# yoraish/mmd

Hardware: AMD Instinct MI355X
Metric: guided trajectories/sec (H=64, 100 denoise steps), 32-robot Empty map (higher is better)
Workload: dtype f32 (f16x2 split on the fp16 MFMA pipe: every fp32 product as 3 fp16 MFMAs, fp32 accumulate)

## Files before the change

### include/mmd_amd.h

```cpp
#ifndef MMD_AMD_H
#define MMD_AMD_H

#include <stddef.h>
#include <stdint.h>

#ifdef __cplusplus
extern "C" {
#endif

#define MMD_AMD_ABI_VERSION 9
#define MMD_STATE_DIM 4
#define MMD_HORIZON 64

typedef struct mmd_unet_s* mmd_unet_t;

int mmd_abi_version(void);
const char* mmd_last_error(void);


int mmd_unet_num_tensors(int unet_input_dim, int n_levels);
int64_t mmd_unet_tensor_numel(int unet_input_dim, int n_levels, int index);

typedef struct mmd_unet_options {
  uint32_t flags;
// ... 17 lines not shown
int mmd_unet_forward(mmd_unet_t unet, const float* x_dev, int t, float* eps_dev, int n_traj, void* workspace_dev,
                     size_t workspace_bytes, void* stream);


typedef struct mmd_cons_bins {
  float lo[2], inv_cell[2];
  int32_t nx, ny, n_all, robot0;
  float radius, weight;
  const int32_t* cell_off_dev;
  const float* entries_dev;
} mmd_cons_bins;

typedef struct mmd_guide_desc {
  float norm_min[MMD_STATE_DIM];
  float norm_max[MMD_STATE_DIM];
  float limits_lo[2];
  float limits_hi[2];
  int32_t grid_nx, grid_ny, n_grids, n_maps;
  const float* sdf_grids_dev;
  const int32_t* robot_map_dev;
  float ws_min[2];
  float ws_max[2];
  float margin;
  float dt;
  float sigma_gp;
  float weight_collision;
  float weight_smoothness;
  float max_grad_norm;
  const float* cons_ell_dev;
  const int32_t* grp_slot_off_dev;
  const float* grp_weight_dev;
  const int32_t* robot_grp_off_dev;
  int32_t max_slots_per_robot;
  float cons_uniform_radius;
  const float* extra_spheres_dev;
  const float* extra_boxes_dev;
  int32_t n_extra_spheres, n_extra_boxes;
  int32_t clip_grad_rule;
  float max_grad_value;
  const mmd_cons_bins* cons_bins;
} mmd_guide_desc;

int mmd_pack_constraints(int n_groups, const int32_t* n_pts, const float* const* q, const float* const* t_range,
                         const float* const* radius, int horizon, float* ell_out, int max_slots,
                         int32_t* slots_out);

int mmd_soft_constraints_from_paths(const float* paths_dev, int n_all, int robot0, int n_local, int horizon,
                                    float radius, float weight, float* ell_out_dev, int32_t* grp_slot_off_dev,
                                    float* grp_weight_dev, int32_t* robot_grp_off_dev, void* stream);

size_t mmd_cons_bins_bytes(int n_all, int nx, int ny, size_t* off_bytes, size_t* entry_bytes);
int mmd_bin_constraints_from_paths(const float* paths_dev, int n_all, int horizon, float radius, const float lo[2], const float hi[2],
                                   int nx, int ny, int32_t* cell_off_dev, float* entries_dev, void* stream);

int mmd_bin_paths(const float* paths_dev, int n_all, int horizon, float reach, const float lo[2], const float hi[2], int nx, int ny,
                  int first_step, int32_t* cell_off_dev, float* entries_dev, void* stream);

int mmd_guide_steps(const mmd_guide_desc* g, float* x_dev, const float* hard_dev, uint64_t hard_rows, int n_robots,
                    int samples_per_robot, int n_steps, float* chain_dev, void* stream);


typedef struct mmd_sampler_desc {
  int32_t n_diffusion_steps;
  const float* sqrt_recip_alphas_cumprod;
  const float* sqrt_recipm1_alphas_cumprod;
  const float* posterior_mean_coef1;
  const float* posterior_mean_coef2;
  const float* posterior_log_variance_clipped;
  int32_t n_guide_steps;
  int32_t t_start_guide;
  float noise_std_extra;
  uint64_t hard_rows;
  int32_t n_streams;
  int64_t traj_index_base;
  const float* noise_std_extra_by_t;
  void* profiler;
  int32_t scale_grad_by_std;
  int32_t model_predicts_x0;
  uint32_t flags;
  int32_t guide_coop_max;
  const uint64_t* robot_seeds_dev;
} mmd_sampler_desc;
#define MMD_SAMPLER_NO_FUSED_STEP 1u
#define MMD_SAMPLER_PERSIST 2u

size_t mmd_sampler_workspace_bytes(mmd_unet_t unet, int n_traj);

int mmd_ddpm_step(mmd_unet_t unet, const mmd_sampler_desc* s, const mmd_guide_desc* guide, float* x_dev,
                  const float* hard_dev, int n_robots, int samples_per_robot, int i, const float* noise_dev,
                  uint64_t seed, uint32_t draw_index, void* workspace_dev, size_t workspace_bytes, void* stream);

int mmd_p_sample_loop(mmd_unet_t unet, const mmd_sampler_desc* s, const mmd_guide_desc* guide, float* x_dev,
                      const float* hard_dev, int n_robots, int samples_per_robot, int n_steps,
                      int n_steps_without_noise, int init_noise, const float* step_noise_dev, uint64_t seed,
                      float* chain_dev, void* workspace_dev, size_t workspace_bytes, void* stream);

int mmd_ddim_sample(mmd_unet_t unet, const mmd_sampler_desc* s, const float* alphas_cumprod, const int32_t* times,
                    int n_times, const mmd_guide_desc* guide, float* x_dev, const float* hard_dev, int n_robots,
                    int samples_per_robot, int init_noise, uint64_t seed, float* chain_dev, void* workspace_dev,
                    size_t workspace_bytes, void* stream);

int mmd_q_sample(float* x_dev, const float* x_start_dev, const float* noise_dev, float sqrt_alphas_cumprod_t,
                 float sqrt_one_minus_alphas_cumprod_t, uint64_t seed, uint32_t draw_index, int64_t traj_index_base,
                 int n_traj, void* stream);

int mmd_cross_condition(float* x1_dev, float* x2_dev, int ind1, int ind2, const float* rel, const float* boundary,
                        int n_traj, void* stream);

typedef struct mmd_ensemble_tile {
  mmd_unet_t unet;
  const mmd_sampler_desc* sampler;
  const mmd_guide_desc* guide;
  float* x_dev;
  const float* hard_dev;
  const float* step_noise_dev;
  float* chain_dev;
  uint64_t seed;
} mmd_ensemble_tile;

typedef struct mmd_cross_cond {
  int32_t m1, m2, ind1, ind2;
  float rel[4];
  float boundary[4];
  const float* by_robot_dev;
} mmd_cross_cond;

int mmd_p_sample_loop_ensemble(const mmd_ensemble_tile* tiles, int n_tiles, const mmd_cross_cond* cross, int n_cross,
                               int n_robots, int samples_per_robot, int n_steps, int n_steps_without_noise,
                               int init_noise, void* workspace_dev, size_t workspace_bytes, void* stream);


int mmd_rr_collisions(const float* paths_dev, int n_robots, int horizon, float margin, uint8_t* mask_dev,
                      float* midpoints_dev, void* stream);

int mmd_count_collisions(const float* trajs_dev, const float* paths_dev, int robot0, int n_local,
                         int samples_per_robot, int n_all, int horizon, float margin, int32_t* counts_dev, void* stream);

int mmd_count_collisions_binned(const float* trajs_dev, const mmd_cons_bins* bins, int n_local, int samples_per_robot, float margin,
                                int32_t* counts_dev, void* stream);

typedef struct mmd_agent_path {
  const float* batch_dev;
  int32_t index;
  int32_t length;
  int32_t start_time;
  int32_t reserved;
} mmd_agent_path;

typedef struct mmd_conflict {
  int32_t t, a, b, reserved;
  float pa[2], pb[2];
  float mid[2];
  float reserved2[2];
} mmd_conflict;

#define MMD_CONFLICTS_ORDERED 0
#define MMD_CONFLICTS_PAIRS 1
#define MMD_SELECT_CBS 0
#define MMD_SELECT_PP 1

int mmd_find_conflicts(const mmd_agent_path* agents_dev, int n_agents, int horizon_global, float margin, int mode,
                       int32_t* row_counts_dev, int32_t* count_dev, mmd_conflict* first_dev, mmd_conflict* list_dev, int list_cap,
                       void* stream);

int mmd_path_conflicts_binned(const float* paths_dev, const mmd_cons_bins* bins, int horizon, float margin, int32_t* row_counts_dev,
                              int32_t* robot_counts_dev, int32_t* count_dev, mmd_conflict* first_dev, mmd_conflict* list_dev, int list_cap,
// ... 62 lines not shown
```

### mmd_amd/_lib.py

```python
import ctypes as C
import os

_HERE = os.path.dirname(os.path.abspath(__file__))
LIB_PATH = os.path.join(_HERE, "lib", "libmmd_amd.so")
ABI_VERSION = 9
HARD_ROWS_START_GOAL = (1 << 63) | 1


def signed64(mask):
    mask = int(mask) & 0xFFFFFFFFFFFFFFFF
    return mask - (1 << 64) if mask >> 63 else mask



class ConsBins(C.Structure):
    _fields_ = [
        ("lo", C.c_float * 2), ("inv_cell", C.c_float * 2),
        ("nx", C.c_int32), ("ny", C.c_int32), ("n_all", C.c_int32), ("robot0", C.c_int32),
        ("radius", C.c_float), ("weight", C.c_float),
        ("cell_off_dev", C.c_void_p), ("entries_dev", C.c_void_p),
    ]


class GuideDesc(C.Structure):
    _fields_ = [
        ("norm_min", C.c_float * 4), ("norm_max", C.c_float * 4),
        ("limits_lo", C.c_float * 2), ("limits_hi", C.c_float * 2),
        ("grid_nx", C.c_int32), ("grid_ny", C.c_int32), ("n_grids", C.c_int32), ("n_maps", C.c_int32),
        ("sdf_grids_dev", C.c_void_p), ("robot_map_dev", C.c_void_p),
        ("ws_min", C.c_float * 2), ("ws_max", C.c_float * 2),
        ("margin", C.c_float), ("dt", C.c_float), ("sigma_gp", C.c_float),
        ("weight_collision", C.c_float), ("weight_smoothness", C.c_float), ("max_grad_norm", C.c_float),
        ("cons_ell_dev", C.c_void_p), ("grp_slot_off_dev", C.c_void_p), ("grp_weight_dev", C.c_void_p),
        ("robot_grp_off_dev", C.c_void_p), ("max_slots_per_robot", C.c_int32), ("cons_uniform_radius", C.c_float),
        ("extra_spheres_dev", C.c_void_p), ("extra_boxes_dev", C.c_void_p),
        ("n_extra_spheres", C.c_int32), ("n_extra_boxes", C.c_int32),
        ("clip_grad_rule", C.c_int32), ("max_grad_value", C.c_float),
        ("cons_bins", C.POINTER(ConsBins)),
    ]


class SamplerDesc(C.Structure):
    _fields_ = [
        ("n_diffusion_steps", C.c_int32),
        ("sqrt_recip_alphas_cumprod", C.POINTER(C.c_float)),
        ("sqrt_recipm1_alphas_cumprod", C.POINTER(C.c_float)),
        ("posterior_mean_coef1", C.POINTER(C.c_float)),
        ("posterior_mean_coef2", C.POINTER(C.c_float)),
        ("posterior_log_variance_clipped", C.POINTER(C.c_float)),
        ("n_guide_steps", C.c_int32), ("t_start_guide", C.c_int32),
        ("noise_std_extra", C.c_float), ("hard_rows", C.c_uint64), ("n_streams", C.c_int32),
        ("traj_index_base", C.c_int64), ("noise_std_extra_by_t", C.POINTER(C.c_float)), ("profiler", C.c_void_p),
        ("scale_grad_by_std", C.c_int32), ("model_predicts_x0", C.c_int32),
        ("flags", C.c_uint32), ("guide_coop_max", C.c_int32), ("robot_seeds_dev", C.c_void_p),
    ]


SAMPLER_NO_FUSED_STEP, SAMPLER_PERSIST = 1, 2
UNET_LAYERED, UNET_LAYERED_VALU = 1, 2
UNET_PRECISION_F32, UNET_PRECISION_F16 = 0, 1
UNET_PRECISIONS = {"f32": UNET_PRECISION_F32, "f16": UNET_PRECISION_F16}


class UnetOptions(C.Structure):
    _fields_ = [("flags", C.c_uint32), ("rtb_fused", C.c_int32), ("mconv_max_cs", C.c_int32), ("two_per_workgroup_max", C.c_int32),
                ("precision", C.c_int32)]


class EnsembleTile(C.Structure):
    _fields_ = [
        ("unet", C.c_void_p), ("sampler", C.POINTER(SamplerDesc)), ("guide", C.POINTER(GuideDesc)),
        ("x_dev", C.c_void_p), ("hard_dev", C.c_void_p), ("step_noise_dev", C.c_void_p), ("chain_dev", C.c_void_p),
        ("seed", C.c_uint64),
    ]


class CrossCond(C.Structure):
    _fields_ = [("m1", C.c_int32), ("m2", C.c_int32), ("ind1", C.c_int32), ("ind2", C.c_int32),
                ("rel", C.c_float * 4), ("boundary", C.c_float * 4), ("by_robot_dev", C.c_void_p)]


class AgentPath(C.Structure):
    _fields_ = [("batch_dev", C.c_void_p), ("index", C.c_int32), ("length", C.c_int32), ("start_time", C.c_int32),
                ("reserved", C.c_int32)]


class Conflict(C.Structure):
    _fields_ = [("t", C.c_int32), ("a", C.c_int32), ("b", C.c_int32), ("reserved", C.c_int32), ("pa", C.c_float * 2),
                ("pb", C.c_float * 2), ("mid", C.c_float * 2), ("reserved2", C.c_float * 2)]


class TileRef(C.Structure):
    _fields_ = [("agent", C.c_int32), ("t0", C.c_int32), ("offset", C.c_float * 2), ("rule", C.c_int32), ("reserved", C.c_int32)]


ADHERENCE_LINE, ADHERENCE_HIGHWAYS, ADHERENCE_CONVEYOR, ADHERENCE_DROP_REGION = 0, 1, 2, 3
CONFLICTS_ORDERED, CONFLICTS_PAIRS = 0, 1
SELECT_CBS, SELECT_PP = 0, 1


_SIGNATURES = {
    "mmd_abi_version": (C.c_int, []),
    "mmd_last_error": (C.c_char_p, []),
    "mmd_unet_num_tensors": (C.c_int, [C.c_int, C.c_int]),
    "mmd_unet_tensor_numel": (C.c_int64, [C.c_int, C.c_int, C.c_int]),
    "mmd_unet_create": (C.c_int, [C.POINTER(C.c_void_p), C.c_int, C.c_int, C.c_int, C.POINTER(C.c_void_p),
                                  C.POINTER(C.c_int64), C.c_int, C.POINTER(UnetOptions), C.c_void_p]),
    "mmd_unet_destroy": (C.c_int, [C.c_void_p]),
    "mmd_unet_workspace_bytes": (C.c_size_t, [C.c_void_p, C.c_int]),
    "mmd_unet_forward": (C.c_int, [C.c_void_p, C.c_void_p, C.c_int, C.c_void_p, C.c_int, C.c_void_p, C.c_size_t,
                                   C.c_void_p]),
    "mmd_pack_constraints": (C.c_int, [C.c_int, C.POINTER(C.c_int32), C.POINTER(C.c_void_p), C.POINTER(C.c_void_p),
                                       C.POINTER(C.c_void_p), C.c_int, C.c_void_p, C.c_int, C.POINTER(C.c_int32)]),
    "mmd_soft_constraints_from_paths": (C.c_int, [C.c_void_p, C.c_int, C.c_int, C.c_int, C.c_int, C.c_float, C.c_float,
                                                  C.c_void_p, C.c_void_p, C.c_void_p, C.c_void_p, C.c_void_p]),
    "mmd_cons_bins_bytes": (C.c_size_t, [C.c_int, C.c_int, C.c_int, C.POINTER(C.c_size_t), C.POINTER(C.c_size_t)]),
    "mmd_bin_constraints_from_paths": (C.c_int, [C.c_void_p, C.c_int, C.c_int, C.c_float, C.POINTER(C.c_float), C.POINTER(C.c_float),
                                                 C.c_int, C.c_int, C.c_void_p, C.c_void_p, C.c_void_p]),
    "mmd_bin_paths": (C.c_int, [C.c_void_p, C.c_int, C.c_int, C.c_float, C.POINTER(C.c_float), C.POINTER(C.c_float), C.c_int, C.c_int,
                                C.c_int, C.c_void_p, C.c_void_p, C.c_void_p]),
    "mmd_guide_steps": (C.c_int, [C.POINTER(GuideDesc), C.c_void_p, C.c_void_p, C.c_uint64, C.c_int, C.c_int, C.c_int,
                                  C.c_void_p, C.c_void_p]),
    "mmd_sampler_workspace_bytes": (C.c_size_t, [C.c_void_p, C.c_int]),
    "mmd_ddpm_step": (C.c_int, [C.c_void_p, C.POINTER(SamplerDesc), C.POINTER(GuideDesc), C.c_void_p, C.c_void_p,
                                C.c_int, C.c_int, C.c_int, C.c_void_p, C.c_uint64, C.c_uint32, C.c_void_p, C.c_size_t,
                                C.c_void_p]),
    "mmd_p_sample_loop": (C.c_int, [C.c_void_p, C.POINTER(SamplerDesc), C.POINTER(GuideDesc), C.c_void_p, C.c_void_p,
                                    C.c_int, C.c_int, C.c_int, C.c_int, C.c_int, C.c_void_p, C.c_uint64, C.c_void_p,
                                    C.c_void_p, C.c_size_t, C.c_void_p]),
    "mmd_ddim_sample": (C.c_int, [C.c_void_p, C.POINTER(SamplerDesc), C.c_void_p, C.c_void_p, C.c_int, C.POINTER(GuideDesc),
                                  C.c_void_p, C.c_void_p, C.c_int, C.c_int, C.c_int, C.c_uint64, C.c_void_p, C.c_void_p,
                                  C.c_size_t, C.c_void_p]),
    "mmd_p_sample_loop_ensemble": (C.c_int, [C.POINTER(EnsembleTile), C.c_int, C.POINTER(CrossCond), C.c_int, C.c_int,
                                             C.c_int, C.c_int, C.c_int, C.c_int, C.c_void_p, C.c_size_t, C.c_void_p]),
    "mmd_q_sample": (C.c_int, [C.c_void_p, C.c_void_p, C.c_void_p, C.c_float, C.c_float, C.c_uint64, C.c_uint32,
                               C.c_int64, C.c_int, C.c_void_p]),
    "mmd_rr_collisions": (C.c_int, [C.c_void_p, C.c_int, C.c_int, C.c_float, C.c_void_p, C.c_void_p, C.c_void_p]),
    "mmd_count_collisions": (C.c_int, [C.c_void_p, C.c_void_p, C.c_int, C.c_int, C.c_int, C.c_int, C.c_int, C.c_float,
                                       C.c_void_p, C.c_void_p]),
    "mmd_count_collisions_binned": (C.c_int, [C.c_void_p, C.POINTER(ConsBins), C.c_int, C.c_int, C.c_float, C.c_void_p, C.c_void_p]),
    "mmd_path_conflicts_binned": (C.c_int, [C.c_void_p, C.POINTER(ConsBins), C.c_int, C.c_float, C.c_void_p, C.c_void_p, C.c_void_p,
# ... 109 lines not shown
```

### mmd_amd/csrc/api.hip

```cpp
#include <hip/hip_runtime.h>

#include <cmath>
#include <cstdarg>
#include <cstdio>
#include <cstdlib>
#include <map>
#include <vector>

#include "../../include/mmd_amd.h"
#include "../../include/mmd_amd_debug.h"
#include "common.h"
#include "guide_dev.h"

struct mmd_profiler_s {
  int stride = 1, window = 1, period = 0;
  std::vector<hipEvent_t> ev;
  std::vector<int> kind;
  hipEvent_t base = nullptr;
  size_t used = 0;
  size_t seen[2] = {0, 0};
};

namespace mmd {

// ... 30 lines not shown
  int nch = n_streams;
  if (nch <= 0) nch = (long long)n_robots * samples_per_robot > 512 ? 2 : 1;
  if (nch > kMaxChunks) nch = kMaxChunks;
  if (nch > n_robots) nch = n_robots;
  return nch < 1 ? 1 : nch;
}


struct Streams {
  hipStream_t s[kMaxChunks] = {};
  hipEvent_t fork = nullptr, join[kMaxChunks] = {};
  bool tried = false, good = false;
  bool ok() {
    if (!tried) {
      tried = true;
      good = hipEventCreateWithFlags(&fork, hipEventDisableTiming) == hipSuccess;
      for (int c = 0; c < kMaxChunks && good; ++c)
        good = hipStreamCreateWithFlags(&s[c], hipStreamNonBlocking) == hipSuccess &&
               hipEventCreateWithFlags(&join[c], hipEventDisableTiming) == hipSuccess;
    }
    return good;
  }
};
static Streams& streams() {
  static thread_local std::map<int, Streams> S;
  int dev = 0;
  (void)hipGetDevice(&dev);
  return S[dev];
}

static StepDev step_base(const mmd_sampler_desc* s) {
  StepDev sd{};
  sd.do_model = 1;
  sd.n_guide_steps = s->n_guide_steps;
  sd.hard_rows = s->hard_rows; sd.n_hard = __builtin_popcountll(s->hard_rows);
  sd.traj_base = (long long)s->traj_index_base;
  return sd;
}

static int make_step(const mmd_sampler_desc* s, int i, bool guided, StepDev& sd) {
  const int t = i < 0 ? 0 : i;
  MMD_REQUIRE(t < s->n_diffusion_steps, "loop index %d outside the %d-step schedule", i, s->n_diffusion_steps);
  sd = step_base(s);
  sd.a_t = s->sqrt_recip_alphas_cumprod[t];
  sd.b_t = s->sqrt_recipm1_alphas_cumprod[t];
  if (s->model_predicts_x0) { sd.a_t = 0.f; sd.b_t = -1.f; }
  sd.grad_scale = s->scale_grad_by_std ? expf(s->posterior_log_variance_clipped[t]) : 1.f;
  sd.c1 = s->posterior_mean_coef1[t];
  sd.c2 = s->posterior_mean_coef2[t];
  sd.sigma = expf(0.5f * s->posterior_log_variance_clipped[t]);
  sd.noise_std_extra = s->noise_std_extra_by_t ? s->noise_std_extra_by_t[t] : s->noise_std_extra;
  sd.do_guide = guided && i < s->t_start_guide ? 1 : 0;
  sd.do_noise = t == 0 ? 0 : 1;
  sd.robot_seeds = reinterpret_cast<const unsigned long long*>(s->robot_seeds_dev);
  sd.coop_max = s->guide_coop_max;
  return 0;
}

static StepDev make_ddim_step(const mmd_sampler_desc* s, const float* alphas_cumprod, int t, int tn, bool guided) {
  StepDev sd = step_base(s);
  sd.ddim = s->model_predicts_x0 ? 2 : 1;
  sd.grad_scale = 1.f;
  sd.a_t = s->sqrt_recip_alphas_cumprod[t];
  sd.b_t = s->model_predicts_x0 ? (tn < 0 ? 0.f : 1.f / s->sqrt_recipm1_alphas_cumprod[t]) : s->sqrt_recipm1_alphas_cumprod[t];
  sd.c1 = tn < 0 ? 1.f : sqrtf(alphas_cumprod[tn]);
  sd.c2 = tn < 0 ? 0.f : sqrtf(1.f - alphas_cumprod[tn]);
  sd.do_guide = guided && tn >= 0 && tn < s->t_start_guide ? 1 : 0;
  sd.do_noise = 0;
  return sd;
}

static FusedStep fused_step(const StepDev& sd, float* x, const float* hard, const float* noise, float* chain, int traj0, int spr,
                            int t_row = 0) {
  FusedStep fs{};
  fs.enabled = 1;
  fs.a_t = sd.a_t; fs.b_t = sd.b_t; fs.c1 = sd.c1; fs.c2 = sd.c2; fs.sigma = sd.sigma; fs.noise_std_extra = sd.noise_std_extra;
  fs.do_noise = sd.do_noise; fs.hard_rows = sd.hard_rows; fs.n_hard = sd.n_hard; fs.seed = sd.seed; fs.draw = sd.draw;
  fs.robot_seeds = sd.robot_seeds;
  fs.traj_base = sd.traj_base; fs.traj0 = traj0; fs.spr = spr;
  fs.x = reinterpret_cast<float4*>(x); fs.noise = reinterpret_cast<const float4*>(noise);
  fs.chain = reinterpret_cast<float4*>(chain); fs.hard = reinterpret_cast<const float4*>(hard);
  fs.t_row = t_row;
  return fs;
}

static int bins_of(const mmd_guide_desc* guide, const mmd_sampler_desc* s, const mmd_cons_bins** out) {
  *out = guide ? guide->cons_bins : nullptr;
  MMD_REQUIRE(!(*out && s->robot_seeds_dev), "cons_bins with per-robot seeds (robot_seeds_dev: batched planner calls) is not supported");
  return 0;
}

template <class T>
static inline T* row_of(T* buf, size_t k, size_t traj_floats) { return buf ? buf + k * traj_floats : nullptr; }

static inline float* eps_of(void* workspace_dev, mmd_unet_t unet, int n) {
  return reinterpret_cast<float*>(reinterpret_cast<char*>(workspace_dev) + mmd_unet_workspace_bytes(unet, n));
}

static int ddpm_step(mmd_unet_t unet, const mmd_sampler_desc* s, const mmd_guide_desc* guide, float* x_dev, const float* hard_dev, int n,
                     int samples_per_robot, int i, const float* noise_dev, uint64_t seed, uint32_t draw_index, void* workspace_dev,
                     mmd_profiler_t prof, float* mu_dev, float* guide_chain_dev, uint32_t* trace_dev, void* stream) {
  StepDev sd{};
  if (int rc = make_step(s, i, guide != nullptr, sd)) return rc;
  sd.seed = seed; sd.draw = draw_index;
  const mmd_cons_bins* bins = nullptr;
  if (int rc = bins_of(guide, s, &bins)) return rc;
  if (trace_dev) {
    MMD_REQUIRE(!bins, "mmd_debug_ddpm_step_trace: the decision dump reads the ELL table, not a cell table (cons_bins)");
    MMD_REQUIRE(sd.do_guide, "mmd_debug_ddpm_step_trace: step %d is not a guided one (t_start_guide %d)", i, s->t_start_guide);
    sd.guide_chain = reinterpret_cast<float4*>(guide_chain_dev);
    sd.guide_chain_stride = (long long)n * H;
    sd.trace = trace_dev;
    sd.mu_out = reinterpret_cast<float4*>(mu_dev);
  }
  GuideDev g{};
  if (sd.do_guide)
    if (int rc = fill_guide(guide, g)) return rc;
  float* eps = eps_of(workspace_dev, unet, n);
  if (int rc = mmd_unet_forward_profiled(unet, x_dev, i < 0 ? 0 : i, eps, n, workspace_dev, mmd_unet_workspace_bytes(unet, n), prof, stream))
    return rc;
  launch_step(g, sd, x_dev, eps, noise_dev, nullptr, hard_dev, 0, n, samples_per_robot, (hipStream_t)stream, bins);
  MMD_HIP_CHECK(hipGetLastError());
  return 0;
}

}

using namespace mmd;

extern "C" {

int mmd_abi_version(void) { return MMD_AMD_ABI_VERSION; }
int mmd_sampler_stream_chunks(int n_streams, int n_robots, int samples_per_robot) {
  return stream_chunks(n_streams, n_robots, samples_per_robot);
}
const char* mmd_last_error(void) { return g_err; }

size_t mmd_sampler_workspace_bytes(mmd_unet_t unet, int n_traj) {
  return mmd_unet_workspace_bytes(unet, n_traj) + (size_t)(n_traj > 0 ? n_traj : 0) * H * D * sizeof(float);
}

int mmd_ddpm_step(mmd_unet_t unet, const mmd_sampler_desc* s, const mmd_guide_desc* guide, float* x_dev,
                  const float* hard_dev, int n_robots, int samples_per_robot, int i, const float* noise_dev,
                  uint64_t seed, uint32_t draw_index, void* workspace_dev, size_t workspace_bytes, void* stream) {
  MMD_REQUIRE(unet && s && x_dev && hard_dev && workspace_dev, "mmd_ddpm_step: NULL argument");
  const int n = n_robots * samples_per_robot;
  MMD_REQUIRE(n >= 1, "mmd_ddpm_step: empty batch");
  MMD_REQUIRE(workspace_bytes >= mmd_sampler_workspace_bytes(unet, n), "mmd_ddpm_step: workspace too small");
  return ddpm_step(unet, s, guide, x_dev, hard_dev, n, samples_per_robot, i, noise_dev, seed, draw_index, workspace_dev,
                   (mmd_profiler_t)s->profiler, nullptr, nullptr, nullptr, stream);
}

int mmd_debug_ddpm_step_trace(mmd_unet_t unet, const mmd_sampler_desc* s, const mmd_guide_desc* guide, float* x_dev,
                              const float* hard_dev, int n_robots, int samples_per_robot, int i, const float* noise_dev,
                              uint64_t seed, uint32_t draw_index, void* workspace_dev, size_t workspace_bytes,
                              float* mu_dev, float* guide_chain_dev, uint32_t* trace_dev, void* stream) {
  MMD_REQUIRE(unet && s && guide && x_dev && hard_dev && workspace_dev && guide_chain_dev && trace_dev,
              "mmd_debug_ddpm_step_trace: NULL argument");
  const int n = n_robots * samples_per_robot;
  MMD_REQUIRE(n >= 1, "mmd_debug_ddpm_step_trace: empty batch");
  MMD_REQUIRE(workspace_bytes >= mmd_sampler_workspace_bytes(unet, n), "mmd_debug_ddpm_step_trace: workspace too small");
  return ddpm_step(unet, s, guide, x_dev, hard_dev, n, samples_per_robot, i, noise_dev, seed, draw_index, workspace_dev, nullptr,
                   mu_dev, guide_chain_dev, trace_dev, stream);
}

int mmd_p_sample_loop(mmd_unet_t unet, const mmd_sampler_desc* s, const mmd_guide_desc* guide, float* x_dev,
                      const float* hard_dev, int n_robots, int samples_per_robot, int n_steps,
                      int n_steps_without_noise, int init_noise, const float* step_noise_dev, uint64_t seed,
                      float* chain_dev, void* workspace_dev, size_t workspace_bytes, void* stream) {
  MMD_REQUIRE(unet && s && x_dev && hard_dev && workspace_dev, "mmd_p_sample_loop: NULL argument");
  const int n = n_robots * samples_per_robot;
  MMD_REQUIRE(n >= 1, "mmd_p_sample_loop: empty batch");
  MMD_REQUIRE(n_steps >= 0 && n_steps <= s->n_diffusion_steps && n_steps_without_noise >= 0, "bad step counts");
  MMD_REQUIRE(workspace_bytes >= mmd_sampler_workspace_bytes(unet, n), "mmd_p_sample_loop: workspace too small");
  hipStream_t st = (hipStream_t)stream;
  const size_t traj_floats = (size_t)n * H * D;
  GuideDev g{};
  if (guide)
    if (int rc = fill_guide(guide, g)) return rc;
  const mmd_cons_bins* bins = nullptr;
  if (int rc = bins_of(guide, s, &bins)) return rc;
  launch_init(x_dev, chain_dev, hard_dev, s->hard_rows, init_noise, (unsigned long long)seed,
              reinterpret_cast<const unsigned long long*>(s->robot_seeds_dev), (long long)s->traj_index_base, n, samples_per_robot, st);
  const bool persist = (s->flags & MMD_SAMPLER_PERSIST) != 0, no_fused_step = (s->flags & MMD_SAMPLER_NO_FUSED_STEP) != 0;
  const mmd_profiler_t prof = (mmd_profiler_t)s->profiler;

  int k_start = 0;
  hipStreamCaptureStatus capturing = hipStreamCaptureStatusNone;
  if (persist) (void)hipStreamIsCapturing(st, &capturing);
  if (persist && capturing == hipStreamCaptureStatusNone && !no_fused_step && unet_fused_step_supported(unet) && !prof) {
    FusedStep run[PERSIST_MAX_STEPS];
    int i = n_steps - 1, k0 = 0;
    while (i >= -n_steps_without_noise) {
      int m = 0;
      for (; m < PERSIST_MAX_STEPS && i - m >= -n_steps_without_noise; ++m) {
        StepDev sd{};
        if (int rc = make_step(s, i - m, guide != nullptr, sd)) return rc;
        if (sd.do_guide) break;
        sd.seed = seed; sd.draw = (unsigned int)(k0 + m);
        run[m] = fused_step(sd, x_dev, hard_dev, row_of(step_noise_dev, k0 + m, traj_floats), row_of(chain_dev, k0 + m + 1, traj_floats), 0,
                            samples_per_robot, i - m < 0 ? 0 : i - m);
      }
      if (m == 0 || (m < 2 && k0 == 0)) break;
      if (int rc = unet_persist_steps(unet, n, workspace_dev, mmd_unet_workspace_bytes(unet, n), st, run, m)) return rc;
      k0 += m; i -= m;
    }
    k_start = k0;
  }
  int nch = stream_chunks(s->n_streams, n_robots, samples_per_robot);
  if (!unet_fused_step_supported(unet)) nch = 1;
  Streams* S = nullptr;
  if (nch > 1) {
    S = &streams();
    if (!S->ok()) nch = 1;
  }
  hipStream_t cs[kMaxChunks];
  int r0[kMaxChunks + 1];
  for (int c = 0; c <= nch; ++c) r0[c] = (int)((long long)n_robots * c / nch);
  for (int c = 0; c < nch; ++c) cs[c] = nch == 1 ? st : S->s[c];
  const size_t uws = mmd_unet_workspace_bytes(unet, n);
  float* eps = eps_of(workspace_dev, unet, n);
  if (nch > 1) {
    MMD_HIP_CHECK(hipEventRecord(S->fork, st));
    for (int c = 0; c < nch; ++c) MMD_HIP_CHECK(hipStreamWaitEvent(cs[c], S->fork, 0));
  }
  int rc = 0, k = k_start;
  for (int i = n_steps - 1 - k_start; i >= -n_steps_without_noise && rc == 0; --i, ++k) {
    StepDev sd{};
    if ((rc = make_step(s, i, guide != nullptr, sd))) break;
    sd.seed = seed; sd.draw = (unsigned int)k;
    const bool fused = !sd.do_guide && !no_fused_step && unet_fused_step_supported(unet);
    const float* noise_k = row_of(step_noise_dev, k, traj_floats);
    float* chain_k = row_of(chain_dev, k + 1, traj_floats);
    for (int c = 0; c < nch && rc == 0; ++c) {
      const int t0 = r0[c] * samples_per_robot, nc = (r0[c + 1] - r0[c]) * samples_per_robot;
      rc = unet_forward_fused(unet, x_dev + (size_t)t0 * H * D, i < 0 ? 0 : i, eps + (size_t)t0 * H * D, nc, workspace_dev, uws, prof, cs[c],
                              fused ? fused_step(sd, x_dev, hard_dev, noise_k, chain_k, t0, samples_per_robot) : FusedStep{});
      if (fused) prof_skip(prof, 1);
    }
    for (int c = 0; c < nch && rc == 0 && !fused; ++c) {
      const int t0 = r0[c] * samples_per_robot, nc = (r0[c + 1] - r0[c]) * samples_per_robot;
      const bool br = prof_begin(prof, 1, sd.do_guide ? MMD_PROF_STEP_GUIDED : MMD_PROF_STEP_PLAIN, cs[c]);
      launch_step(g, sd, x_dev, eps, noise_k, chain_k, hard_dev, t0, nc, samples_per_robot, cs[c], bins);
      if (br) prof_end(prof, cs[c]);
    }
  }
  if (nch > 1)
    for (int c = 0; c < nch; ++c) {
      if (hipEventRecord(S->join[c], cs[c]) != hipSuccess || hipStreamWaitEvent(st, S->join[c], 0) != hipSuccess) {
        if (rc == 0) { set_error("mmd_p_sample_loop: joining side stream %d failed", c); rc = 1; }
      }
    }
  if (rc) return rc;
  MMD_HIP_CHECK(hipGetLastError());
  return 0;
}

int mmd_p_sample_loop_ensemble(const mmd_ensemble_tile* tiles, int n_tiles, const mmd_cross_cond* cross, int n_cross,
                               int n_robots, int samples_per_robot, int n_steps, int n_steps_without_noise,
                               int init_noise, void* workspace_dev, size_t workspace_bytes, void* stream) {
  MMD_REQUIRE(tiles && n_tiles >= 1 && (n_cross == 0 || cross) && workspace_dev, "mmd_p_sample_loop_ensemble: NULL argument");
  const int n = n_robots * samples_per_robot;
  MMD_REQUIRE(n >= 1 && n_steps >= 0 && n_steps_without_noise >= 0, "mmd_p_sample_loop_ensemble: bad sizes");
  hipStream_t st = (hipStream_t)stream;
  const size_t traj_floats = (size_t)n * H * D;
  GuideDev g[8];
  const mmd_cons_bins* bins[8];
  MMD_REQUIRE(n_tiles <= 8, "mmd_p_sample_loop_ensemble: at most 8 tiles");
  for (int m = 0; m < n_tiles; ++m) {
    const mmd_ensemble_tile& T = tiles[m];
    MMD_REQUIRE(T.unet && T.sampler && T.x_dev && T.hard_dev, "tile %d: NULL member", m);
    MMD_REQUIRE(n_steps <= T.sampler->n_diffusion_steps, "tile %d: more steps than its schedule has", m);
    MMD_REQUIRE(workspace_bytes >= mmd_sampler_workspace_bytes(T.unet, n), "mmd_p_sample_loop_ensemble: workspace too small");
    g[m] = GuideDev{};
    if (T.guide)
      if (int rc = fill_guide(T.guide, g[m])) return rc;
    if (int rc = bins_of(T.guide, T.sampler, &bins[m])) return rc;
  }
  for (int c = 0; c < n_cross; ++c)
    MMD_REQUIRE(cross[c].m1 >= 0 && cross[c].m1 < n_tiles && cross[c].m2 >= 0 && cross[c].m2 < n_tiles &&
                    cross[c].ind1 >= 0 && cross[c].ind1 < H && cross[c].ind2 >= 0 && cross[c].ind2 < H,
                "cross condition %d out of range", c);
  auto cross_all = [&](int crow, int stepped) {
    for (int c = 0; c < n_cross; ++c) {
      const mmd_cross_cond& C = cross[c];
      auto row = [&](int m) { return row_of(tiles[m].chain_dev, m > stepped ? crow - 1 : crow, traj_floats); };
      launch_cross(tiles[C.m1].x_dev, tiles[C.m2].x_dev, row(C.m1), row(C.m2), C.ind1, C.ind2, C.rel, C.boundary, C.by_robot_dev,
                   samples_per_robot, n, st);
    }
  };
  for (int m = 0; m < n_tiles; ++m)
    launch_init(tiles[m].x_dev, tiles[m].chain_dev, tiles[m].hard_dev, tiles[m].sampler->hard_rows, init_noise,
                (unsigned long long)tiles[m].seed, reinterpret_cast<const unsigned long long*>(tiles[m].sampler->robot_seeds_dev),
                (long long)tiles[m].sampler->traj_index_base, n, samples_per_robot, st);
  cross_all(0, n_tiles);
  int k = 0;
  for (int i = n_steps - 1; i >= -n_steps_without_noise; --i, ++k) {
    for (int m = 0; m < n_tiles; ++m) {
      const mmd_ensemble_tile& T = tiles[m];
      StepDev sd{};
      if (int rc = make_step(T.sampler, i, T.guide != nullptr, sd)) return rc;
      sd.seed = T.seed; sd.draw = (unsigned int)k;
      const mmd_profiler_t prof = (mmd_profiler_t)T.sampler->profiler;
      const size_t uws = mmd_unet_workspace_bytes(T.unet, n);
      float* eps = eps_of(workspace_dev, T.unet, n);
      const float* noise_k = row_of(T.step_noise_dev, k, traj_floats);
      float* chain_k = row_of(T.chain_dev, k + 1, traj_floats);
      const bool fused = !sd.do_guide && !(T.sampler->flags & MMD_SAMPLER_NO_FUSED_STEP) && unet_fused_step_supported(T.unet);
      if (int rc = unet_forward_fused(T.unet, T.x_dev, i < 0 ? 0 : i, eps, n, workspace_dev, uws, prof, st,
                                      fused ? fused_step(sd, T.x_dev, T.hard_dev, noise_k, chain_k, 0, samples_per_robot) : FusedStep{}))
        return rc;
      if (!fused) launch_step(g[m], sd, T.x_dev, eps, noise_k, chain_k, T.hard_dev, 0, n, samples_per_robot, st, bins[m]);
      cross_all(k + 1, m);
    }
  }
  MMD_HIP_CHECK(hipGetLastError());
  return 0;
}

int mmd_ddim_sample(mmd_unet_t unet, const mmd_sampler_desc* s, const float* alphas_cumprod, const int32_t* times,
                    int n_times, const mmd_guide_desc* guide, float* x_dev, const float* hard_dev, int n_robots,
                    int samples_per_robot, int init_noise, uint64_t seed, float* chain_dev, void* workspace_dev,
                    size_t workspace_bytes, void* stream) {
// ... 104 lines not shown
```

### mmd_amd/csrc/guide.hip

```cpp
#include <hip/hip_runtime.h>

#include <algorithm>
#include <atomic>
#include <cmath>
#include <cstdlib>
#include <cstring>
#include <vector>

#include "../../include/mmd_amd.h"
#include "../../include/mmd_amd_debug.h"
#include "bins_dev.h"
#include "common.h"
#include "guide_dev.h"

namespace mmd {

__device__ __forceinline__ float clip_scale(float gx, float gy, float gz, float gw, float max_norm) {
  const float ax = gx + 1e-6f, ay = gy + 1e-6f, az = gz + 1e-6f, aw = gw + 1e-6f;
  const float n2 = ax * ax + ay * ay + az * az + aw * aw;
  return fminf(max_norm * __builtin_amdgcn_rsqf(n2), 1.f);
}

__device__ __forceinline__ bool clip_grad(const GuideDev& g, float& gx, float& gy, float& gz, float& gw) {
  if (g.clip_rule == 0) {
    const float sc = clip_scale(gx, gy, gz, gw, g.max_norm);
    gx = sc * gx; gy = sc * gy; gz = sc * gz; gw = sc * gw;
    return sc < 1.f;
  } else if (g.clip_rule == 1) {
    const float m = g.max_value;
    const bool on = fabsf(gx) > m || fabsf(gy) > m || fabsf(gz) > m || fabsf(gw) > m;
    gx = fminf(fmaxf(gx, -m), m); gy = fminf(fmaxf(gy, -m), m); gz = fminf(fmaxf(gz, -m), m); gw = fminf(fmaxf(gw, -m), m);
    return on;
  }
  return false;
}
__device__ __forceinline__ bool clip_grad(const GuideDev& g, float& gx, float& gy) {
  float z = 0.f, w = 0.f;
  return clip_grad(g, gx, gy, z, w);
}

__device__ __forceinline__ float lane_prev(float v) {
  return __builtin_bit_cast(float, __builtin_amdgcn_update_dpp(0, __builtin_bit_cast(int, v), 0x138, 0xf, 0xf, true));
}
__device__ __forceinline__ float lane_next(float v) {
  return __builtin_bit_cast(float, __builtin_amdgcn_update_dpp(0, __builtin_bit_cast(int, v), 0x130, 0xf, 0xf, true));
}

constexpr int LDS_SLOTS_SMALL = 40;
constexpr int LDS_SLOTS_MAX = 144;

__device__ __forceinline__ float rsq_pos(float d2) { return __builtin_amdgcn_rsqf(fmaxf(d2, 1e-30f)); }

typedef float f32x2g __attribute__((ext_vector_type(2)));
struct Acc4 { f32x2g a0, a1, a2, a3; };
__device__ __forceinline__ Acc4 acc4_zero() {
  const f32x2g z = {0.f, 0.f};
  return Acc4{z, z, z, z};
}
__device__ __forceinline__ f32x2g acc4_total(const Acc4& r) {
  return f32x2g{(r.a0.x + r.a1.x) + (r.a2.x + r.a3.x), (r.a0.y + r.a1.y) + (r.a2.y + r.a3.y)};
}
__device__ __forceinline__ f32x2g cons_term(f32x2g a, f32x2g p, f32x2g q, float r2) {
  const float dx = p.x - q.x, dy = p.y - q.y;
  const float d2 = __builtin_fmaf(dx, dx, dy * dy);
  const float m = (d2 > r2) ? 0.f : rsq_pos(d2);
  return f32x2g{__builtin_fmaf(-dx, m, a.x), __builtin_fmaf(-dy, m, a.y)};
}
template <bool COMPACT> struct ConsTab;
template <> struct ConsTab<false> {
  const float4* tab;
  float r2;
  __device__ __forceinline__ f32x2g add(f32x2g a, f32x2g p, int slot, int t) const {
    const float4 c = tab[slot * H + t];
    return cons_term(a, p, f32x2g{c.x, c.y}, c.w);
  }
};
template <> struct ConsTab<true> {
  const float2* tab;
  float r2;
  __device__ __forceinline__ f32x2g add(f32x2g a, f32x2g p, int slot, int t) const {
    const float2 c = tab[slot * H + t];
    return cons_term(a, p, f32x2g{c.x, c.y}, r2);
  }
};
template <class TAB>
__device__ __forceinline__ void cons_accumulate4(Acc4& acc, const TAB& tab, int first, int n, int rel, int t, f32x2g p) {
  auto one = [&](int k, int slot) {
    if (k == 0) acc.a0 = tab.add(acc.a0, p, slot, t);
    else if (k == 1) acc.a1 = tab.add(acc.a1, p, slot, t);
    else if (k == 2) acc.a2 = tab.add(acc.a2, p, slot, t);
    else acc.a3 = tab.add(acc.a3, p, slot, t);
  };
  int i = 0;
  for (; i < n && ((rel + i) & 3); ++i) one((rel + i) & 3, first + i);
#pragma unroll 2
  for (; i + 3 < n; i += 4) {
    acc.a0 = tab.add(acc.a0, p, first + i, t);
    acc.a1 = tab.add(acc.a1, p, first + i + 1, t);
    acc.a2 = tab.add(acc.a2, p, first + i + 2, t);
    acc.a3 = tab.add(acc.a3, p, first + i + 3, t);
  }
  for (int k = 0; i < n; ++i, ++k) one(k, first + i);
}
template <class TAB>
__device__ __forceinline__ f32x2g cons_accumulate1(f32x2g a, const TAB& tab, int first, int n, int rel, int k, int t, f32x2g p) {
#pragma unroll 4
  for (int j = (k - rel) & 3; j < n; j += 4) a = tab.add(a, p, first + j, t);
  return a;
}

struct GroupMeta {
  static constexpr bool kOneGroup = false;
  int s0[2], s1[2];
  float w[2];
  int grp0, n;
  __device__ __forceinline__ void load(const GuideDev& g, int g0, int g1) {
    grp0 = g0;
    n = min(g1 - g0, 2);
#pragma unroll
    for (int k = 0; k < 2; ++k) {
      s0[k] = s1[k] = 0;
      w[k] = 0.f;
      if (k < n) {
        s0[k] = __builtin_amdgcn_readfirstlane(g.grp_slot_off[g0 + k]);
        s1[k] = __builtin_amdgcn_readfirstlane(g.grp_slot_off[g0 + k + 1]);
        w[k] = __builtin_bit_cast(float, __builtin_amdgcn_readfirstlane(__builtin_bit_cast(int, g.grp_weight[g0 + k])));
      }
    }
  }
  __device__ __forceinline__ void bounds(const GuideDev& g, int grp, int& a, int& b) const {
    const int k = grp - grp0;
    if (k == 0 && n > 0) { a = s0[0]; b = s1[0]; }
    else if (k == 1 && n > 1) { a = s0[1]; b = s1[1]; }
    else { a = __builtin_amdgcn_readfirstlane(g.grp_slot_off[grp]); b = __builtin_amdgcn_readfirstlane(g.grp_slot_off[grp + 1]); }
  }
  __device__ __forceinline__ float weight(const GuideDev& g, int grp) const {
    const int k = grp - grp0;
    return (k == 0 && n > 0) ? w[0] : (k == 1 && n > 1) ? w[1] : g.grp_weight[grp];
  }
};

template <bool DUMP = false, class GROUPSUM, class GROUPW>
__device__ __forceinline__ float4 guide_grad(const GuideDev& g, float4 xn, int t, const float4* __restrict__ grid,
                                             int grp0, int grp1, GROUPSUM group_sum, GROUPW group_weight, unsigned int* tr = nullptr) {
  unsigned int flags = 0;
  float xu[4];
  const float xv[4] = {xn.x, xn.y, xn.z, xn.w};
#pragma unroll
  for (int d = 0; d < 4; ++d) {
    float v = fminf(fmaxf(xv[d], -1.f), 1.f);
    if constexpr (DUMP) flags |= (fabsf(xv[d]) > 1.f ? 1u : 0u) << (16 + d);
    v = (v + 1.f) / 2.f;
    xu[d] = v * g.nscale[d] + g.nmin[d];
  }
  const float px = xu[0], py = xu[1], vx = xu[2], vy = xu[3];
  const bool interior = t > 0 && t < H - 1;

  int ix = (int)floorf((px - g.lo[0]) / g.dim[0] * (float)g.nx);
  int iy = (int)floorf((py - g.lo[1]) / g.dim[1] * (float)g.ny);
  ix = min(max(ix, 0), g.nx - 1);
  iy = min(max(iy, 0), g.ny - 1);
  const float4 cell0 = g.n_grids > 0 ? grid[(size_t)ix * g.ny + iy] : make_float4(1e30f, 0.f, 0.f, 0.f);

  float wsx, wsy;
  {
    const float d0 = px - g.ws_min[0], d1 = py - g.ws_min[1], d2 = g.ws_max[0] - px, d3 = g.ws_max[1] - py;
    float best = fmaxf(g.margin - d0, 0.f), gx = -1.f, gy = 0.f;
    float v = fmaxf(g.margin - d1, 0.f);
    if (v > best) { best = v; gx = 0.f; gy = -1.f; }
    v = fmaxf(g.margin - d2, 0.f);
    if (v > best) { best = v; gx = 1.f; gy = 0.f; }
    v = fmaxf(g.margin - d3, 0.f);
    if (v > best) { best = v; gx = 0.f; gy = 1.f; }
    if (!(best > 0.f)) { gx = 0.f; gy = 0.f; }
    if constexpr (DUMP) {
      const unsigned arg = gx < 0.f ? 0u : gy < 0.f ? 1u : gx > 0.f ? 2u : 3u;
      if (best > 0.f) flags |= 1u << 4 | arg << 5;
    }
    const bool clipped = clip_grad(g, gx, gy);
    if constexpr (DUMP) flags |= (clipped ? 1u : 0u) << 9;
    wsx = g.w_coll * gx; wsy = g.w_coll * gy;
  }
  float gpx, gpy, gpz, gpw;
  {
    const float npx = lane_next(px), npy = lane_next(py), nvx = lane_next(vx), nvy = lane_next(vy);
    float wpx = 0.f, wpy = 0.f, wvx = 0.f, wvy = 0.f;
    if (t < H - 1) {
      const float epx = npx - (px + g.dt * vx), epy = npy - (py + g.dt * vy);
      const float evx = nvx - vx, evy = nvy - vy;
      wpx = 2.f * (g.m1 * epx + g.m2 * evx);
      wpy = 2.f * (g.m1 * epy + g.m2 * evy);
      wvx = 2.f * (g.m2 * epx + g.m3 * evx);
      wvy = 2.f * (g.m2 * epy + g.m3 * evy);
    }
    const float lpx = lane_prev(wpx), lpy = lane_prev(wpy), lvx = lane_prev(wvx), lvy = lane_prev(wvy);
    float gx = lpx - wpx, gy = lpy - wpy;
    float gz = lvx - (g.dt * wpx + wvx), gw = lvy - (g.dt * wpy + wvy);
    const bool clipped = clip_grad(g, gx, gy, gz, gw);
    if constexpr (DUMP) flags |= (clipped ? 1u : 0u) << 10;
    gpx = g.w_smooth * gx; gpy = g.w_smooth * gy;
    gpz = g.w_smooth * gz; gpw = g.w_smooth * gw;
  }
  float cx = 0.f, cy = 0.f;
  for (int grp = grp0; grp < grp1; ++grp) {
    const f32x2g gs = group_sum(grp, f32x2g{px, py});
    float gx = gs.x, gy = gs.y;
    const bool clipped = clip_grad(g, gx, gy);
    if constexpr (DUMP) {
      const int k = grp - grp0, s0 = g.grp_slot_off[grp], s1 = g.grp_slot_off[grp + 1];
      unsigned long long mask = 0;
      unsigned int n_act = 0;
      for (int sl = s0; sl < s1; ++sl) {
        const float4 c = g.cons[(size_t)sl * H + t];
        const float dx = px - c.x, dy = py - c.y;
        const float d2 = __builtin_fmaf(dx, dx, dy * dy);
        if (!(d2 > c.w)) {
          ++n_act;
          if (sl - s0 < 64) mask |= 1ull << (sl - s0);
        }
      }
      if (k < 4) {
        tr[2 + 2 * k] = (unsigned int)mask;
        tr[3 + 2 * k] = (unsigned int)(mask >> 32);
        flags |= (clipped ? 1u : 0u) << (11 + k);
      }
      tr[10] += n_act;
    }
    const float w = group_weight(grp);
    cx += w * gx; cy += w * gy;
  }
  float ox, oy;
  {
    float best = fmaxf(g.margin - cell0.x, 0.f), gx = 0.f, gy = 0.f;
    unsigned win = 0;
    if (best > 0.f) { gx = -cell0.y; gy = -cell0.z; }
    for (int k = 1; k < g.n_grids; ++k) {
      const float4 c = grid[((size_t)k * g.nx + ix) * g.ny + iy];
      const float v = fmaxf(g.margin - c.x, 0.f);
      if (v > best) { best = v; gx = -c.y; gy = -c.z; win = (unsigned)k; }
    }
    if (g.n_xs + g.n_xb > 0) {
      float ex, ey;
      const float v = fmaxf(g.margin - extra_sdf(g.xs, g.n_xs, g.xb, g.n_xb, px, py, ex, ey), 0.f);
      if (v > best) { best = v; gx = -ex; gy = -ey; win = 7u; }
    }
    const bool clipped = clip_grad(g, gx, gy);
    if constexpr (DUMP) {
      if (best > 0.f) flags |= 1u | (win & 7u) << 1;
      flags |= (clipped ? 1u : 0u) << 8;
    }
    ox = g.w_coll * gx; oy = g.w_coll * gy;
  }
  if constexpr (DUMP) {
    tr[0] = (unsigned int)(ix * g.ny + iy);
    tr[1] = flags | (unsigned int)min(grp1 - grp0, 15) << 20;
  }
  float tx = ((ox + wsx) + gpx) + cx, ty = ((oy + wsy) + gpy) + cy;
  float tz = gpz, tw = gpw;
  if (!interior) { tx = ty = tz = tw = 0.f; }
  return make_float4(-tx, -ty, -tz, -tw);
}


template <bool COMPACT, int NT>
__device__ __forceinline__ void stage_cons(const GuideDev& g, int robot, int lds_slots, float4* lds_cons, int& lds_slot0, int& lds_n) {
  lds_slot0 = __builtin_amdgcn_readfirstlane(g.grp_slot_off[g.robot_grp_off[robot]]);
  lds_n = min(__builtin_amdgcn_readfirstlane(g.grp_slot_off[g.robot_grp_off[robot + 1]]) - lds_slot0, lds_slots);
  const float4* src = g.cons + (size_t)lds_slot0 * H;
  if constexpr (COMPACT) {
    float2* dst = reinterpret_cast<float2*>(lds_cons);
    for (int i = threadIdx.x; i < lds_n * H; i += NT) {
      const float4 c = src[i];
      dst[i] = c.z < 0.f ? make_float2(1e30f, 1e30f) : make_float2(c.x, c.y);
    }
  } else {
    for (int i = threadIdx.x; i < lds_n * H; i += NT) lds_cons[i] = src[i];
  }
}

template <bool COMPACT, class ACC>
__device__ __forceinline__ void group_slots(const GuideDev& g, const GroupMeta& gm, int grp, const float4* lds_cons, int lds_slot0, int lds_n,
                                            ACC acc) {
  int s0, s1;
  gm.bounds(g, grp, s0, s1);
  const int l0 = min(max(s0 - lds_slot0, 0), lds_n), l1 = min(max(s1 - lds_slot0, 0), lds_n);
  if (l1 > l0) {
    if constexpr (COMPACT) acc(ConsTab<true>{reinterpret_cast<const float2*>(lds_cons), g.uniform_r2}, l0, l1 - l0, lds_slot0 + l0 - s0);
    else acc(ConsTab<false>{lds_cons, 0.f}, l0, l1 - l0, lds_slot0 + l0 - s0);
  }
  const int g0 = lds_n > 0 ? max(s0, lds_slot0 + lds_n) : s0;
  if (s1 > g0) acc(ConsTab<false>{g.cons, 0.f}, g0, s1 - g0, g0 - s0);
}

__device__ __forceinline__ float4 model_update(StepDev s, float4 v, const float4* eps, size_t idx) {
  if (s.do_model)
    v = s.ddim == 2 ? ddim_update_x0(v, eps[idx], s.a_t, s.b_t, s.c1, s.c2)
        : s.ddim ? ddim_update(v, eps[idx], s.a_t, s.b_t, s.c1, s.c2) : ddpm_posterior_mean(v, eps[idx], s.a_t, s.b_t, s.c1, s.c2);
  return v;
}

template <bool DUMP, class META = GroupMeta, class GROUPSUM>
__device__ __forceinline__ void guide_iterations(const GuideDev& g, const StepDev& s, int robot, int t, size_t idx, float4& v, bool is_hard,
                                                 float4 hv, bool store, GROUPSUM group_sum) {
  const int map = g.robot_map ? g.robot_map[robot] : 0;
  const float4* grid = g.grids + (size_t)map * g.n_grids * g.nx * g.ny;
  int grp0 = 0, grp1 = 0;
  if constexpr (META::kOneGroup) {
    grp1 = 1;
  } else if (g.robot_grp_off) {
    grp0 = __builtin_amdgcn_readfirstlane(g.robot_grp_off[robot]);
    grp1 = __builtin_amdgcn_readfirstlane(g.robot_grp_off[robot + 1]);
  }
  META gm;
  if constexpr (META::kOneGroup) gm.w = group_sum.weight;
  gm.load(g, grp0, grp1);
  for (int it = 0; it < s.n_guide_steps; ++it) {
    unsigned int* tr = nullptr;
    if constexpr (DUMP) {
      tr = s.trace + ((size_t)it * s.guide_chain_stride + idx) * MMD_TRACE_WORDS;
      for (int w = 0; w < MMD_TRACE_WORDS; ++w) tr[w] = 0u;
    }
    const float4 gr = guide_grad<DUMP>(g, v, t, grid, grp0, grp1, [&](int grp, f32x2g p) { return group_sum(gm, grp, p); },
                                       [&](int grp) { return gm.weight(g, grp); }, tr);
    v.x = __builtin_fmaf(s.grad_scale, gr.x, v.x); v.y = __builtin_fmaf(s.grad_scale, gr.y, v.y);
    v.z = __builtin_fmaf(s.grad_scale, gr.z, v.z); v.w = __builtin_fmaf(s.grad_scale, gr.w, v.w);
    if (is_hard) v = hv;
    if (s.guide_chain && store) s.guide_chain[(size_t)it * s.guide_chain_stride + idx] = v;
  }
}

__device__ __forceinline__ void step_finish(const StepDev& s, float4* x, const float4* noise, float4* chain, size_t idx, int robot,
                                            int samples_per_robot, float4& v, bool is_hard, const float4& hv) {
  if (s.do_noise) v = add_step_noise(v, noise ? noise[idx] : traj_normal4(s.seed, s.robot_seeds, s.draw, s.traj_base, idx, robot, samples_per_robot), s.sigma, s.noise_std_extra);
  if (is_hard) v = hv;
  x[idx] = v;
  if (chain) chain[idx] = v;
}

template <int WPB, bool COMPACT, bool DUMP = false>
__global__ __launch_bounds__(WPB * 64) void ddpm_guide_kernel(GuideDev g, StepDev s, int lds_slots, float4* __restrict__ x,
                                                         const float4* __restrict__ eps,
                                                         const float4* __restrict__ noise, float4* __restrict__ chain,
                                                         const float4* __restrict__ hard,
                                                         int samples_per_robot) {
  extern __shared__ __attribute__((aligned(16))) float4 lds_cons[];
  const int t = threadIdx.x & 63;
  const int traj_b = s.traj0 + blockIdx.x * WPB;
  const int traj = traj_b + (threadIdx.x >> 6);
  const bool valid = traj < s.traj_end;

  int lds_slot0 = 0, lds_n = 0;
  if (s.do_guide && g.robot_grp_off) {
    const int rb0 = traj_b / samples_per_robot;
    const int rb1 = min(traj_b + WPB - 1, s.traj_end - 1) / samples_per_robot;
    if (rb0 == rb1) stage_cons<COMPACT, WPB * 64>(g, rb0, lds_slots, lds_cons, lds_slot0, lds_n);
  }
  __syncthreads();
  if (!valid) return;

  const int robot = traj / samples_per_robot;
  const size_t idx = (size_t)traj * H + t;
  float4 v = model_update(s, x[idx], eps, idx);
  float4 hv = v;
  const bool is_hard = hard_row(s.hard_rows, s.n_hard, hard, robot, t, hv);
  if constexpr (DUMP) {
    if (s.mu_out) s.mu_out[idx] = v;
  }
  if (s.do_guide)
    guide_iterations<DUMP>(g, s, robot, t, idx, v, is_hard, hv, true, [&](const GroupMeta& gm, int grp, f32x2g p) {
      Acc4 acc = acc4_zero();
      group_slots<COMPACT>(g, gm, grp, lds_cons, lds_slot0, lds_n,
                           [&](const auto& tab, int first, int n, int rel) { cons_accumulate4(acc, tab, first, n, rel, t, p); });
      return acc4_total(acc);
    });
  step_finish(s, x, noise, chain, idx, robot, samples_per_robot, v, is_hard, hv);
}

constexpr int COOP_XCH_BYTES = 2 * 4 * H * 8;
template <bool COMPACT>
__global__ __launch_bounds__(256) void ddpm_guide_coop_kernel(GuideDev g, StepDev s, int lds_slots, float4* __restrict__ x,
                                                              const float4* __restrict__ eps, const float4* __restrict__ noise,
                                                              float4* __restrict__ chain, const float4* __restrict__ hard,
                                                              int samples_per_robot) {
  extern __shared__ __attribute__((aligned(16))) float4 lds_cons[];
  const int t = threadIdx.x & 63, wave = __builtin_amdgcn_readfirstlane(threadIdx.x >> 6);
  const int traj = s.traj0 + blockIdx.x;
  const int robot = traj / samples_per_robot;
  float2* const xch = reinterpret_cast<float2*>(reinterpret_cast<char*>(lds_cons) + (size_t)lds_slots * H * (COMPACT ? 8 : 16));
  int lds_slot0 = 0, lds_n = 0;
  if (s.do_guide && g.robot_grp_off) stage_cons<COMPACT, 256>(g, robot, lds_slots, lds_cons, lds_slot0, lds_n);
  __syncthreads();
  const size_t idx = (size_t)traj * H + t;
  float4 v = model_update(s, x[idx], eps, idx);
  float4 hv = v;
  const bool is_hard = hard_row(s.hard_rows, s.n_hard, hard, robot, t, hv);
  if (s.do_guide) {
    int parity = 0;
    guide_iterations<false>(g, s, robot, t, idx, v, is_hard, hv, wave == 0, [&](const GroupMeta& gm, int grp, f32x2g p) {
      f32x2g a = {0.f, 0.f};
      group_slots<COMPACT>(g, gm, grp, lds_cons, lds_slot0, lds_n,
                           [&](const auto& tab, int first, int n, int rel) { a = cons_accumulate1(a, tab, first, n, rel, wave, t, p); });
      float2* const slot = xch + parity * 4 * H;
      slot[wave * H + t] = make_float2(a.x, a.y);
      __syncthreads();
      parity ^= 1;
      const float2 q0 = slot[t], q1 = slot[H + t], q2 = slot[2 * H + t], q3 = slot[3 * H + t];
      return acc4_total(Acc4{f32x2g{q0.x, q0.y}, f32x2g{q1.x, q1.y}, f32x2g{q2.x, q2.y}, f32x2g{q3.x, q3.y}});
    });
  }
  if (wave != 0) return;
  step_finish(s, x, noise, chain, idx, robot, samples_per_robot, v, is_hard, hv);
}


struct OneGroup {
  static constexpr bool kOneGroup = true;
  float w;
  __device__ __forceinline__ void load(const GuideDev&, int, int) {}
  __device__ __forceinline__ float weight(const GuideDev&, int) const { return w; }
// ... 136 lines not shown
    lds_cell[r] = bin_cell(p.x, lo0, inv0, nx) << 16 | bin_cell(p.y, lo1, inv1, ny);
  }
  __syncthreads();
  const int cpt = (ncell + BIN_THREADS - 1) / BIN_THREADS;
  const int c0 = min(tid * cpt, ncell), c1 = min(c0 + cpt, ncell);
  auto near = [&](int rc, int ix, int iy) { return abs((rc >> 16) - ix) <= 1 && abs((rc & 0xffff) - iy) <= 1; };
  int cnt = 0;
  for (int c = c0; c < c1; ++c) {
    const int ix = c / ny, iy = c - ix * ny;
    for (int r = 0; r < n_all; ++r) cnt += near(lds_cell[r], ix, iy) ? 1 : 0;
  }
  scan[tid] = cnt;
  __syncthreads();
  for (int d = 1; d < BIN_THREADS; d <<= 1) {
    const int add = tid >= d ? scan[tid - d] : 0;
    __syncthreads();
    scan[tid] += add;
    __syncthreads();
  }
  int pos = scan[tid] - cnt;
  float4* const seg = entries + (size_t)t * 9 * n_all;
  for (int c = c0; c < c1; ++c) {
    const int ix = c / ny, iy = c - ix * ny;
    off[c] = pos;
    for (int r = 0; r < n_all; ++r)
      if (near(lds_cell[r], ix, iy)) {
        const float2 p = lds_pts[r];
        seg[pos++] = make_float4(p.x, p.y, __builtin_bit_cast(float, r), 0.f);
      }
  }
  if (tid == BIN_THREADS - 1) off[ncell] = scan[tid];
}

constexpr int BIN_MAX_ROBOTS = 4096;
constexpr int BIN_MAX_CELLS = 64;

int check_cons_bins(const mmd_cons_bins* b) {
  MMD_REQUIRE(b->cell_off_dev && b->entries_dev, "cons_bins: NULL table");
  MMD_REQUIRE(b->nx >= 1 && b->nx <= BIN_MAX_CELLS && b->ny >= 1 && b->ny <= BIN_MAX_CELLS, "cons_bins: grid %d x %d outside [1, %d]", b->nx,
              b->ny, BIN_MAX_CELLS);
  MMD_REQUIRE(b->n_all >= 2 && b->robot0 >= 0 && b->robot0 < b->n_all, "cons_bins: bad robot range");
  MMD_REQUIRE(b->radius > 0.f, "cons_bins: radius must be positive");
  for (int k = 0; k < 2; ++k)
    MMD_REQUIRE(b->inv_cell[k] > 0.f && 1.0 / (double)b->inv_cell[k] >= 1.0625 * (double)b->radius * (1.0 - 1e-6),
                "cons_bins: cells smaller than (1 + 1/16) x the radius");
  return 0;
}

int fill_guide(const mmd_guide_desc* d, GuideDev& g) {
  MMD_REQUIRE(d->n_grids == 0 || (d->sdf_grids_dev && d->grid_nx >= 1 && d->grid_ny >= 1), "guide: SDF grid missing");
  if (d->cons_bins) {
    MMD_REQUIRE(!d->cons_ell_dev, "guide: cons_bins together with an ELL table (cons_ell_dev) is not supported");
    if (int rc = check_cons_bins(d->cons_bins)) return rc;
  }
  for (int k = 0; k < 4; ++k) { g.nmin[k] = d->norm_min[k]; g.nscale[k] = d->norm_max[k] - d->norm_min[k]; }
  for (int k = 0; k < 2; ++k) {
    g.lo[k] = d->limits_lo[k];
    g.dim[k] = fabsf(d->limits_hi[k] - d->limits_lo[k]);
    g.ws_min[k] = d->ws_min[k]; g.ws_max[k] = d->ws_max[k];
  }
  g.nx = d->grid_nx; g.ny = d->grid_ny; g.n_grids = d->n_grids;
  g.grids = reinterpret_cast<const float4*>(d->sdf_grids_dev);
  g.robot_map = d->robot_map_dev;
  g.margin = d->margin; g.dt = d->dt; g.w_coll = d->weight_collision; g.w_smooth = d->weight_smoothness;
  g.max_norm = d->max_grad_norm;
  MMD_REQUIRE(d->clip_grad_rule >= 0 && d->clip_grad_rule <= 2, "guide: clip_grad_rule must be 0 (norm), 1 (value) or 2 (off)");
  g.clip_rule = d->clip_grad_rule;
  g.max_value = d->max_grad_value;
  const double dt = d->dt, qc = 1.0 / ((double)d->sigma_gp * d->sigma_gp);
  g.m1 = (float)(12.0 / (dt * dt * dt) * qc);
  g.m2 = (float)(-6.0 / (dt * dt) * qc);
  g.m3 = (float)(4.0 / dt * qc);
  g.max_slots = d->max_slots_per_robot > 0 ? d->max_slots_per_robot : LDS_SLOTS_SMALL;
  g.uniform_r2 = d->cons_uniform_radius > 0.f ? d->cons_uniform_radius * fabsf(d->cons_uniform_radius) : 0.f;
  g.xs = reinterpret_cast<const float4*>(d->extra_spheres_dev); g.n_xs = d->extra_spheres_dev ? d->n_extra_spheres : 0;
  g.xb = reinterpret_cast<const float4*>(d->extra_boxes_dev); g.n_xb = d->extra_boxes_dev ? d->n_extra_boxes : 0;
  g.cons = reinterpret_cast<const float4*>(d->cons_ell_dev);
  g.grp_slot_off = d->grp_slot_off_dev; g.grp_weight = d->grp_weight_dev; g.robot_grp_off = d->robot_grp_off_dev;
  if (!g.cons || !g.grp_slot_off || !g.grp_weight) g.robot_grp_off = nullptr;
  return 0;
}

constexpr int kCoopMaxTrajDefault = 512;

int launch_step(const GuideDev& g, StepDev s, float* x, const float* eps, const float* noise, float* chain,
                const float* hard, int traj0, int n_traj, int spr, hipStream_t st, const mmd_cons_bins* bins) {
  s.traj0 = traj0;
  s.traj_end = traj0 + n_traj;
  if (bins && s.do_guide) {
    hipLaunchKernelGGL(ddpm_guide_binned_kernel, dim3((n_traj + 3) / 4), dim3(256), 0, st, g, s, *bins, (float4*)x, (const float4*)eps,
                       (const float4*)noise, (float4*)chain, (const float4*)hard, spr);
    return 0;
  }
  const bool guided = s.do_guide && g.robot_grp_off;
  const bool compact = guided && g.uniform_r2 > 0.f;
  const int bytes_per_slot = H * (compact ? 8 : 16);
  const int small = LDS_SLOTS_SMALL * (compact ? 2 : 1), big = LDS_SLOTS_MAX * (compact ? 2 : 1);
  auto launch = [&](auto kern, int grid, int block, size_t lds_bytes, int slots) {
    hipLaunchKernelGGL(kern, dim3(grid), dim3(block), lds_bytes, st, g, s, slots, (float4*)x, (const float4*)eps, (const float4*)noise,
                       (float4*)chain, (const float4*)hard, spr);
  };
  if (s.trace) {
    launch(ddpm_guide_kernel<4, false, true>, (n_traj + 3) / 4, 256, 0, 0);
  } else if (guided && n_traj <= (s.coop_max > 0 ? s.coop_max : s.coop_max < 0 ? 0 : kCoopMaxTrajDefault)) {
    const int fit = 60 * 1024 / bytes_per_slot;
    const int slots = g.max_slots < fit ? g.max_slots : fit;
    launch(compact ? ddpm_guide_coop_kernel<true> : ddpm_guide_coop_kernel<false>, n_traj, 256,
           (size_t)slots * bytes_per_slot + COOP_XCH_BYTES, slots);
  } else if (guided && g.max_slots > small && spr % 8 == 0 && traj0 % 8 == 0) {
    const int slots = g.max_slots < big ? g.max_slots : big;
    static std::atomic<unsigned long long> attr_devices{0};
    int dev = 0;
    (void)hipGetDevice(&dev);
    const unsigned long long bit = 1ull << (dev & 63);
    if (!(attr_devices.load(std::memory_order_acquire) & bit)) {
      (void)hipFuncSetAttribute(reinterpret_cast<const void*>(&ddpm_guide_kernel<8, false>),
                                hipFuncAttributeMaxDynamicSharedMemorySize, LDS_SLOTS_MAX * H * 16);
      (void)hipFuncSetAttribute(reinterpret_cast<const void*>(&ddpm_guide_kernel<8, true>),
                                hipFuncAttributeMaxDynamicSharedMemorySize, LDS_SLOTS_MAX * H * 16);
      attr_devices.fetch_or(bit, std::memory_order_release);
    }
    launch(compact ? ddpm_guide_kernel<8, true> : ddpm_guide_kernel<8, false>, (n_traj + 7) / 8, 512, (size_t)slots * bytes_per_slot, slots);
  } else {
    const int slots = guided ? small : 0;
    launch(compact ? ddpm_guide_kernel<4, true> : ddpm_guide_kernel<4, false>, (n_traj + 3) / 4, 256, (size_t)slots * bytes_per_slot, slots);
  }
  return 0;
}

void launch_cross(float* x1, float* x2, float* c1, float* c2, int ind1, int ind2, const float* rel, const float* bnd,
                  const float* by_robot, int spr, int n_traj, hipStream_t st) {
  hipLaunchKernelGGL(cross_condition_kernel, dim3((n_traj + 255) / 256), dim3(256), 0, st, (float4*)x1, (float4*)x2,
                     (float4*)c1, (float4*)c2, ind1, ind2, make_float4(rel[0], rel[1], rel[2], rel[3]),
                     make_float4(bnd[0], bnd[1], bnd[2], bnd[3]), (const float4*)by_robot, spr > 0 ? spr : 1, n_traj);
}

int launch_init(float* x, float* chain, const float* hard, unsigned long long hard_rows, int draw, unsigned long long seed,
                const unsigned long long* robot_seeds, long long traj_base, int n_traj, int spr, hipStream_t st) {
  const size_t n = (size_t)n_traj * H;
  hipLaunchKernelGGL(init_kernel, dim3((unsigned)((n + 255) / 256)), dim3(256), 0, st, (float4*)x, (float4*)chain,
                     (const float4*)hard, hard_rows, draw, seed, robot_seeds, traj_base, n_traj, spr);
  return 0;
}

}

using namespace mmd;

extern "C" {

int mmd_pack_constraints(int n_groups, const int32_t* n_pts, const float* const* q, const float* const* t_range,
                         const float* const* radius, int horizon, float* ell_out, int max_slots, int32_t* slots_out) {
  MMD_REQUIRE(horizon == H, "mmd_pack_constraints: horizon must be %d", H);
  int used = 0;
  for (int g = 0; g < n_groups; ++g) {
    std::vector<int> fill(H, 0);
    for (int c = 0; c < n_pts[g]; ++c) {
      const int t0 = (int)ceilf(t_range[g][2 * c]), t1 = (int)ceilf(t_range[g][2 * c + 1]);
      for (int t = t0 < 0 ? 0 : t0; t < t1 && t < H; ++t) ++fill[t];
    }
    int slots = 0;
    for (int t = 0; t < H; ++t) slots = fill[t] > slots ? fill[t] : slots;
    slots_out[g] = slots;
    if (!ell_out) { used += slots; continue; }
    MMD_REQUIRE(used + slots <= max_slots, "mmd_pack_constraints: need more than %d slots", max_slots);
    for (int s = 0; s < slots; ++s)
      for (int t = 0; t < H; ++t) {
        float* e = ell_out + ((size_t)(used + s) * H + t) * 4;
        e[0] = 0.f; e[1] = 0.f; e[2] = -1.f; e[3] = -1.f;
      }
    std::fill(fill.begin(), fill.end(), 0);
    for (int c = 0; c < n_pts[g]; ++c) {
      const int t0 = (int)ceilf(t_range[g][2 * c]), t1 = (int)ceilf(t_range[g][2 * c + 1]);
      for (int t = t0 < 0 ? 0 : t0; t < t1 && t < H; ++t) {
        float* e = ell_out + ((size_t)(used + fill[t]) * H + t) * 4;
        e[0] = q[g][2 * c]; e[1] = q[g][2 * c + 1]; e[2] = radius[g][c];
        e[3] = radius[g][c] * fabsf(radius[g][c]);
        ++fill[t];
      }
    }
    used += slots;
  }
  return 0;
}

int mmd_soft_constraints_from_paths(const float* paths_dev, int n_all, int robot0, int n_local, int horizon,
                                    float radius, float weight, float* ell_out_dev, int32_t* grp_slot_off_dev,
// ... 94 lines not shown
```

### mmd_amd/csrc/guide_dev.h

```cpp
#pragma once
#include <hip/hip_runtime.h>

#include "../../include/mmd_amd.h"
#include "common.h"

namespace mmd {

struct GuideDev {
  float nmin[4], nscale[4];
  float lo[2], dim[2];
  int nx, ny, n_grids;
  const float4* grids;
  const int* robot_map;
  float ws_min[2], ws_max[2];
  float margin, dt, w_coll, w_smooth, max_norm;
  int clip_rule;
  float max_value;
  float m1, m2, m3;
  const float4* cons;
  const int* grp_slot_off;
  const float* grp_weight;
  const int* robot_grp_off;
  int max_slots;
  float uniform_r2;
  const float4* xs;
  const float4* xb;
  int n_xs, n_xb;
};

template <bool kTorchNorm = false>
__device__ __forceinline__ float extra_sdf(const float4* __restrict__ xs, int n_xs, const float4* __restrict__ xb, int n_xb,
                                           float px, float py, float& gx, float& gy) {
  float best = n_xs + n_xb > 0 ? 1e30f : 1.f;
  gx = 0.f; gy = 0.f;
  for (int i = 0; i < n_xs; ++i) {
    const float4 s = xs[i];
    const float dx = px - s.x, dy = py - s.y;
    const float n = kTorchNorm ? sqrtf(__builtin_fmaf(dy, dy, dx * dx)) : sqrtf(dx * dx + dy * dy), d = n - s.z;
    if (d < best) { best = d; gx = n > 0.f ? dx / n : 0.f; gy = n > 0.f ? dy / n : 0.f; }
  }
  for (int i = 0; i < n_xb; ++i) {
    const float4 b = xb[i];
    const float rad = 0.3f * fminf(b.z, b.w);
    const float dx = px - b.x, dy = py - b.y, qx = fabsf(dx) - b.z + rad, qy = fabsf(dy) - b.w + rad;
    const float mq = fmaxf(qx, qy), rx = fmaxf(qx, 0.f), ry = fmaxf(qy, 0.f);
    const float n = kTorchNorm ? sqrtf(__builtin_fmaf(ry, ry, rx * rx)) : sqrtf(rx * rx + ry * ry);
    const float d = fminf(mq, 0.f) + n - rad;
    if (d < best) {
      best = d;
      const float sx = dx > 0.f ? 1.f : (dx < 0.f ? -1.f : 0.f), sy = dy > 0.f ? 1.f : (dy < 0.f ? -1.f : 0.f);
      if (mq <= 0.f) {
        gx = qx >= qy ? sx : 0.f;
        gy = qx >= qy ? 0.f : sy;
      } else {
        gx = rx / n * sx;
        gy = ry / n * sy;
      }
    }
  }
  return best;
}

__device__ __forceinline__ void philox4x32(unsigned int (&c)[4], unsigned int k0, unsigned int k1) {
#pragma unroll
  for (int r = 0; r < 10; ++r) {
    const unsigned long long p0 = (unsigned long long)0xD2511F53u * c[0];
    const unsigned long long p1 = (unsigned long long)0xCD9E8D57u * c[2];
    const unsigned int n0 = (unsigned int)(p1 >> 32) ^ c[1] ^ k0;
    const unsigned int n1 = (unsigned int)p1;
    const unsigned int n2 = (unsigned int)(p0 >> 32) ^ c[3] ^ k1;
    const unsigned int n3 = (unsigned int)p0;
    c[0] = n0; c[1] = n1; c[2] = n2; c[3] = n3;
    k0 += 0x9E3779B9u; k1 += 0xBB67AE85u;
  }
}

__device__ __forceinline__ float4 normal4(unsigned long long seed, unsigned int draw, unsigned long long point) {
  unsigned int c[4] = {(unsigned int)point, draw, (unsigned int)(point >> 32), 0u};
  philox4x32(c, (unsigned int)seed, (unsigned int)(seed >> 32));
  const float s = 2.3283064365386963e-10f;
  const float u0 = ((float)c[0] + 0.5f) * s, u1 = ((float)c[1] + 0.5f) * s;
  const float u2 = ((float)c[2] + 0.5f) * s, u3 = ((float)c[3] + 0.5f) * s;
  const float r0 = sqrtf(-2.f * logf(u0)), r1 = sqrtf(-2.f * logf(u2));
  float s0, c0, s1, c1;
  sincosf(6.283185307179586f * u1, &s0, &c0);
  sincosf(6.283185307179586f * u3, &s1, &c1);
  return make_float4(r0 * c0, r0 * s0, r1 * c1, r1 * s1);
}

__device__ __forceinline__ float4 traj_normal4(unsigned long long seed, const unsigned long long* robot_seeds, unsigned int draw,
                                               long long traj_base, size_t idx, int robot, int spr) {
  if (robot_seeds) return normal4(robot_seeds[robot], draw, (unsigned long long)(idx - (size_t)robot * spr * H));
  return normal4(seed, draw, (unsigned long long)traj_base * H + idx);
}

__device__ __forceinline__ float ddpm_mean1(float x, float e, float a, float b, float c1, float c2) {
  const float x0 = fminf(fmaxf(__builtin_fmaf(a, x, -(b * e)), -1.f), 1.f);
  return __builtin_fmaf(c1, x0, c2 * x);
}
__device__ __forceinline__ float4 ddpm_posterior_mean(float4 v, float4 e, float a, float b, float c1, float c2) {
  return make_float4(ddpm_mean1(v.x, e.x, a, b, c1, c2), ddpm_mean1(v.y, e.y, a, b, c1, c2), ddpm_mean1(v.z, e.z, a, b, c1, c2),
                     ddpm_mean1(v.w, e.w, a, b, c1, c2));
}
__device__ __forceinline__ float4 ddim_update(float4 v, float4 e, float a, float b, float c1, float c2) {
  auto f = [&](float x, float ee) { return __builtin_fmaf(c1, __builtin_fmaf(a, x, -(b * ee)), c2 * ee); };
  return make_float4(f(v.x, e.x), f(v.y, e.y), f(v.z, e.z), f(v.w, e.w));
}
__device__ __forceinline__ float4 ddim_update_x0(float4 v, float4 o, float a, float b_inv, float c1, float c2) {
  auto f = [&](float x, float oo) { return __builtin_fmaf(c1, oo, c2 * (__builtin_fmaf(a, x, -oo) * b_inv)); };
  return make_float4(f(v.x, o.x), f(v.y, o.y), f(v.z, o.z), f(v.w, o.w));
}
__device__ __forceinline__ float4 add_step_noise(float4 v, float4 z, float sigma, float noise_std_extra) {
  return make_float4(__builtin_fmaf(sigma * z.x, noise_std_extra, v.x), __builtin_fmaf(sigma * z.y, noise_std_extra, v.y),
                     __builtin_fmaf(sigma * z.z, noise_std_extra, v.z), __builtin_fmaf(sigma * z.w, noise_std_extra, v.w));
}

struct FusedStep {
  int enabled;
  float a_t, b_t, c1, c2, sigma, noise_std_extra;
  int do_noise, n_hard;
  unsigned long long hard_rows;
  unsigned long long seed;
  const unsigned long long* robot_seeds;
  unsigned int draw;
  long long traj_base;
  int traj0, spr;
  float4* x;
  const float4* noise;
  float4* chain;
  const float4* hard;
  int t_row;
};

constexpr int PERSIST_MAX_STEPS = 64;
constexpr int PERSIST_ARGS_OFF = 8192;
constexpr int PERSIST_TABLE_BYTES = 12288;
static_assert(PERSIST_MAX_STEPS * sizeof(FusedStep) <= PERSIST_ARGS_OFF, "the step table fits its workspace region");

__device__ __forceinline__ bool hard_row(unsigned long long rows, int n_hard, const float4* hard, int robot, int t, float4& hv) {
  const bool on = (rows >> t) & 1ull;
  if (on) hv = hard[robot * n_hard + __popcll(rows & ((1ull << t) - 1ull))];
  return on;
}

struct StepDev {
  float a_t, b_t, c1, c2;
  float sigma;
  float noise_std_extra;
  float grad_scale;
  int do_model, do_guide, do_noise;
  int ddim;
  int n_guide_steps;
  int n_hard;
  unsigned long long hard_rows;
  unsigned long long seed;
  const unsigned long long* robot_seeds;
  int coop_max;
  unsigned int draw;
  int traj0, traj_end;
  float4* guide_chain;
  long long guide_chain_stride;
  long long traj_base;
  unsigned int* trace;
  float4* mu_out;
};

int fill_guide(const mmd_guide_desc* d, GuideDev& g);
bool unet_fused_step_supported(mmd_unet_t u);
int unet_forward_fused(mmd_unet_t u, const float* x, int t, float* eps, int n, void* ws, size_t ws_bytes, Profiler* prof,
                       hipStream_t st, const FusedStep& fs);
int unet_persist_steps(mmd_unet_t u, int n, void* ws, size_t ws_bytes, hipStream_t st, const FusedStep* steps, int n_steps);
int launch_unet_f16(int ns, int blocks, hipStream_t st, const void* args, size_t args_bytes);
int launch_unet_persist_f16(int ns, int blocks, hipStream_t st, const void* args_dev, size_t args_bytes, const FusedStep* steps_dev,
                            int n_steps, int tb_total);
int launch_step(const GuideDev& g, StepDev s, float* x, const float* eps, const float* noise, float* chain,
                const float* hard, int traj0, int n_traj, int spr, hipStream_t st, const mmd_cons_bins* bins);
int launch_init(float* x, float* chain, const float* hard, unsigned long long hard_rows, int draw, unsigned long long seed,
                const unsigned long long* robot_seeds, long long traj_base, int n_traj, int spr, hipStream_t st);

void launch_cross(float* x1, float* x2, float* c1, float* c2, int ind1, int ind2, const float* rel, const float* bnd,
                  const float* by_robot, int spr, int n_traj, hipStream_t st);

}
```

### mmd_amd/csrc/unet.hip

```cpp
#include <hip/hip_runtime.h>

#include <cmath>
#include <cstring>
#include <memory>
#include <vector>

#include "../../include/mmd_amd.h"
#include "../../include/mmd_amd_debug.h"
#include "common.h"
#include "f16x2.h"
#include "guide_dev.h"
#include "unet_kernel.h"
#include "unet_spec.h"

namespace mmd {

__device__ __forceinline__ float mish_exact(float y) {
  float sp = y > 20.f ? y : log1pf(expf(y));
  return y * tanhf(sp);
}

__global__ void time_table_kernel(TimeArgs a) {
  __shared__ float emb[32], h1[128], m[32];
  const int t = blockIdx.x, tid = threadIdx.x;
// ... 222 lines not shown
    p.fin_is1 = push_inverse(blob, sc1, p.fin_act);
    std::vector<float> w1(16 * 32, 0.f);
    memcpy(w1.data(), tensors[s.t_final[4]], sizeof(float) * 4 * 32);
    sc1.resize(16, 1.f);
    p.fin_w1 = pack_rd(blob, w1.data(), 16, 32, 0, 32, 1, taps1, false, false, sc1);
    p.fin_b1 = push(blob, tensors[s.t_final[5]], 4);
  }
}

static int fill_time_table(const mmd_unet_s* u, const Spec& s, hipStream_t st) {
  const UnetPack& p = u->w;
  TimeArgs ta{};
  ta.w1 = u->blob + p.raw_time[0]; ta.b1 = u->blob + p.raw_time[1];
  ta.w3 = u->blob + p.raw_time[2]; ta.b3 = u->blob + p.raw_time[3];
  for (int r = 0; r < 12; ++r) {
    ta.cw[r] = u->blob + p.raw_cw[r]; ta.cb[r] = u->blob + p.raw_cb[r];
    ta.cout[r] = s.rtb[r].cout; ta.off[r] = p.rtb[r].tb_off;
  }
  ta.n_rtb = 12; ta.total = p.tb_total; ta.table = u->ttable;
  launch_time_table(ta, u->T, st);
  MMD_HIP_CHECK(hipGetLastError());
  MMD_HIP_CHECK(hipStreamSynchronize(st));
  return 0;
}

static RtbPtrs rtb_ptrs(const mmd_unet_s* u, const RtbW& w, int t) {
  RtbPtrs p{};
  p.ba = u->blob + w.a.bias; p.ga = u->blob + w.a.gamma; p.bea = u->blob + w.a.beta;
  p.tb = u->ttable + (size_t)t * u->w.tb_total + w.tb_off;
  p.bb = u->blob + w.b.bias; p.gb = u->blob + w.b.gamma; p.beb = u->blob + w.b.beta;
  p.wa_bf = w.a.wbf ? reinterpret_cast<const uint4*>(u->blob + w.a.wbf) : nullptr;
  p.wb_bf = w.b.wbf ? reinterpret_cast<const uint4*>(u->blob + w.b.wbf) : nullptr;
  p.isa = w.a.wbf ? u->blob + w.a.isc : nullptr;
  p.isb = w.b.wbf ? u->blob + w.b.isc : nullptr;
  p.act_a = w.act_a;
  return p;
}

static ChainArgs args_chain(const mmd_unet_s* u, const int* rtb, int n_ident, const TailW* tail, const float* in0, int t, int n) {
  ChainArgs a{};
  a.in0 = in0; a.n = n;
  const RtbW& w0 = u->w.rtb[rtb[0]];
  a.r0 = rtb_ptrs(u, w0, t);
  a.wa0_c1_bf = w0.a_c1_bf ? reinterpret_cast<const uint4*>(u->blob + w0.a_c1_bf) : nullptr;
  a.br = u->blob + w0.res_bias;
  a.isr = w0.res_isc ? u->blob + w0.res_isc : nullptr;
  a.wres_bf = w0.res_bf ? reinterpret_cast<const uint4*>(u->blob + w0.res_bf) : nullptr;
  a.wres_c1_bf = w0.res_c1_bf ? reinterpret_cast<const uint4*>(u->blob + w0.res_c1_bf) : nullptr;
  for (int k = 0; k < n_ident; ++k) a.ri[k] = rtb_ptrs(u, u->w.rtb[rtb[1 + k]], t);
  if (tail) {
    a.bt = u->blob + tail->bias;
    a.wt_bf0 = reinterpret_cast<const uint4*>(u->blob + tail->wbf[0]);
    a.ist0 = u->blob + tail->isc[0];
    if (tail->wbf[1]) {
      a.wt_bf1 = reinterpret_cast<const uint4*>(u->blob + tail->wbf[1]);
      a.ist1 = u->blob + tail->isc[1];
    }
  }
  return a;
}

static UnetArgs unet_args(const mmd_unet_s* u, const float* x, int t, int n, float* eps) {
  static const int kD0[] = {0, 1}, kD1[] = {2, 3}, kD2[] = {4, 5, 10, 11}, kU0[] = {6, 7}, kU1[] = {8, 9};
  const UnetPack& p = u->w;
  UnetArgs a{};
  a.n = n;
  a.c[0] = args_chain(u, kD0, 1, &p.down[0], x, t, n);
  a.c[1] = args_chain(u, kD1, 1, &p.down[1], nullptr, t, n);
  a.c[2] = args_chain(u, kD2, 3, nullptr, nullptr, t, n);
  a.c[3] = args_chain(u, kU0, 1, &p.up[0], nullptr, t, n);
  a.c[4] = args_chain(u, kU1, 1, &p.up[1], nullptr, t, n);
  a.fin.out = eps;
  a.fin.w5 = reinterpret_cast<const uint4*>(u->blob + p.fin.wbf);
  a.fin.isc = u->blob + p.fin.isc;
  a.fin.bias = u->blob + p.fin.bias; a.fin.gamma = u->blob + p.fin.gamma; a.fin.beta = u->blob + p.fin.beta;
  a.fin.act = p.fin_act;
  a.fin.w1_bf = reinterpret_cast<const uint4*>(u->blob + p.fin_w1);
  a.fin.is1 = u->blob + p.fin_is1;
  a.fin.w1_bias = u->blob + p.fin_b1;
  return a;
}

int unet_forward_fused(mmd_unet_t u, const float* x, int t, float* eps, int n, void* ws, size_t ws_bytes, Profiler* prof,
                       hipStream_t st, const FusedStep& fs) {
  MMD_REQUIRE(u && x && eps && ws, "mmd_unet_forward: NULL argument");
  MMD_REQUIRE(n >= 1, "mmd_unet_forward: n_traj must be >= 1");
  MMD_REQUIRE(t >= 0 && t < u->T, "mmd_unet_forward: t=%d outside [0,%d)", t, u->T);
  MMD_REQUIRE(ws_bytes >= mmd_unet_workspace_bytes(u, n), "mmd_unet_forward: workspace too small");
  if (u->layered) {
    MMD_REQUIRE(!fs.enabled, "mmd_unet_forward: the fused unguided step exists in the fused kernel only");
    const bool bracket = prof_begin(prof, 0, MMD_PROF_UNET, st);
    const int rc = layered_forward(u->layered, x, t, eps, n, ws, ws_bytes, st);
    if (bracket) prof_end(prof, st);
    return rc;
  }
  UnetArgs a = unet_args(u, x, t, n, eps);
  a.fs = fs;
  const bool bracket = prof_begin(prof, 0, fs.enabled ? MMD_PROF_UNET_FUSED : MMD_PROF_UNET, st);
  int rc = 0;
  if (u->precision == MMD_UNET_PRECISION_F16) {
    const int ns = n <= u->ns1_max && n <= u->ns2_max ? 1 : n <= u->ns2_max ? 2 : 4;
    rc = launch_unet_f16(ns, (n + ns - 1) / ns, st, &a, sizeof(a));
  } else if (n <= u->ns1_max && n <= u->ns2_max) hipLaunchKernelGGL(unet_kernel<1>, dim3(n), dim3(256), 0, st, a);
  else if (n <= u->ns2_max) hipLaunchKernelGGL(unet_kernel<2>, dim3((n + 1) / 2), dim3(256), 0, st, a);
  else hipLaunchKernelGGL(unet_kernel<4>, dim3((n + 3) / 4), dim3(256), 0, st, a);
  if (bracket) prof_end(prof, st);
  if (rc) return rc;
  MMD_HIP_CHECK(hipGetLastError());
  return 0;
}

int unet_persist_steps(mmd_unet_t u, int n, void* ws, size_t ws_bytes, hipStream_t st, const FusedStep* steps, int n_steps) {
  MMD_REQUIRE(u && !u->layered && ws && n >= 1, "unet_persist_steps: bad arguments");
  MMD_REQUIRE(n_steps >= 1 && n_steps <= PERSIST_MAX_STEPS && ws_bytes >= (size_t)PERSIST_TABLE_BYTES, "unet_persist_steps: step table");
  for (int s = 0; s < n_steps; ++s) MMD_REQUIRE(steps[s].t_row >= 0 && steps[s].t_row < u->T, "unet_persist_steps: t outside the time table");
  MMD_HIP_CHECK(hipMemcpyAsync(ws, steps, sizeof(FusedStep) * n_steps, hipMemcpyHostToDevice, st));
  char* const args_dev = reinterpret_cast<char*>(ws) + PERSIST_ARGS_OFF;
  const UnetArgs a = unet_args(u, reinterpret_cast<const float*>(steps[0].x), 0, n, nullptr);
  MMD_HIP_CHECK(hipMemcpyAsync(args_dev, &a, sizeof(a), hipMemcpyHostToDevice, st));
  const FusedStep* sd = reinterpret_cast<const FusedStep*>(ws);
  const UnetArgs* ap = reinterpret_cast<const UnetArgs*>(args_dev);
  if (u->precision == MMD_UNET_PRECISION_F16) {
    const int ns = n <= u->ns2_max ? 2 : 4;
    if (int rc = launch_unet_persist_f16(ns, (n + ns - 1) / ns, st, args_dev, sizeof(a), sd, n_steps, u->w.tb_total)) return rc;
  } else if (n <= u->ns2_max) hipLaunchKernelGGL(unet_persist_kernel<2>, dim3((n + 1) / 2), dim3(256), 0, st, ap, sd, n_steps, u->w.tb_total);
  else hipLaunchKernelGGL(unet_persist_kernel<4>, dim3((n + 3) / 4), dim3(256), 0, st, ap, sd, n_steps, u->w.tb_total);
  MMD_HIP_CHECK(hipGetLastError());
  return 0;
}
bool unet_fused_step_supported(mmd_unet_t u) { return u && !u->layered; }

static constexpr double rtb_flops(double cin, double cout, double L) {
  return 2.0 * cout * 5 * cin * L + 2.0 * cout * 5 * cout * L + (cin != cout ? 2.0 * cout * cin * L : 0.0);
}
static const double kUnetFlops =
    rtb_flops(4, 32, 64) + rtb_flops(32, 32, 64) + 2.0 * 32 * 3 * 32 * 32 +
    rtb_flops(32, 64, 32) + rtb_flops(64, 64, 32) + 2.0 * 64 * 3 * 64 * 16 +
    rtb_flops(64, 128, 16) + 3 * rtb_flops(128, 128, 16) +
    rtb_flops(256, 64, 16) + rtb_flops(64, 64, 16) + 2.0 * 64 * 4 * 64 * 16 +
    rtb_flops(128, 32, 32) + rtb_flops(32, 32, 32) + 2.0 * 32 * 4 * 32 * 32 +
    2.0 * 32 * 5 * 32 * 64 + 2.0 * 4 * 32 * 64;

static constexpr double d5(double cin, double cout, double L) { return 2.0 * cout * 5 * cin * L; }
static const double kF16Flops =
    2 * (2.0 * 32 * 32 * 64) + 3 * d5(32, 32, 64) + 2.0 * 32 * 3 * 32 * 32 +
    d5(32, 64, 32) + 2.0 * 64 * 32 * 32 + 3 * d5(64, 64, 32) + 2.0 * 64 * 3 * 64 * 16 +
    d5(64, 128, 16) + 2.0 * 128 * 64 * 16 + 7 * d5(128, 128, 16) +
    d5(256, 64, 16) + 2.0 * 64 * 256 * 16 + 3 * d5(64, 64, 16) + 2.0 * 64 * 4 * 64 * 16 +
    d5(128, 32, 32) + 2.0 * 32 * 128 * 32 + 3 * d5(32, 32, 32) + 2.0 * 32 * 4 * 32 * 32 +
    d5(32, 32, 64) + 2.0 * 16 * 32 * 64;
static const double kFp32Flops = 0.0;
static const double kUnetMfmaFlops = kF16Flops + kFp32Flops;
}

extern "C" {

int mmd_unet_num_tensors(int unet_input_dim, int n_levels) {
  Spec s;
  if (!build_spec(unet_input_dim, n_levels, s)) {
    set_error("unsupported TemporalUnet configuration (unet_input_dim=%d, n_levels=%d)", unet_input_dim, n_levels);
    return -1;
  }
  return (int)s.numel.size();
}

int64_t mmd_unet_tensor_numel(int unet_input_dim, int n_levels, int index) {
  Spec s;
  if (!build_spec(unet_input_dim, n_levels, s) || index < 0 || index >= (int)s.numel.size()) return -1;
  return s.numel[index];
}

int mmd_unet_create(mmd_unet_t* out, int unet_input_dim, int n_levels, int n_diffusion_steps,
                    const float* const* tensors, const int64_t* numels, int n_tensors, const mmd_unet_options* options,
                    void* stream) {
  Spec s;
  MMD_REQUIRE(out != nullptr, "mmd_unet_create: out is NULL");
  MMD_REQUIRE(build_spec(unet_input_dim, n_levels, s),
              "unsupported TemporalUnet configuration (unet_input_dim=%d, n_levels=%d)", unet_input_dim, n_levels);
  MMD_REQUIRE(n_tensors == (int)s.numel.size(), "expected %d parameter tensors, got %d", (int)s.numel.size(), n_tensors);
  for (int i = 0; i < n_tensors; ++i)
    MMD_REQUIRE(numels[i] == s.numel[i] && tensors[i] != nullptr, "parameter tensor %d has %lld elements, expected %lld",
                i, (long long)numels[i], (long long)s.numel[i]);
  MMD_REQUIRE(n_diffusion_steps >= 1, "n_diffusion_steps must be >= 1");
  const int precision = options ? options->precision : MMD_UNET_PRECISION_F32;
  const bool layered_path = !fused_config(unet_input_dim, n_levels) || (options && (options->flags & MMD_UNET_LAYERED));
  MMD_REQUIRE(precision == MMD_UNET_PRECISION_F32 || precision == MMD_UNET_PRECISION_F16,
              "mmd_unet_options.precision = %d: MMD_UNET_PRECISION_F32 (0) or MMD_UNET_PRECISION_F16 (1)", precision);
  MMD_REQUIRE(precision == MMD_UNET_PRECISION_F32 || !layered_path,
              "mmd_unet_options.precision = MMD_UNET_PRECISION_F16 exists in the fused kernel only (unet_input_dim 32, 3 levels, "
              "without MMD_UNET_LAYERED): unet_input_dim=%d, n_levels=%d, flags=%u", unet_input_dim, n_levels, options->flags);
  hipStream_t st = (hipStream_t)stream;

  struct Destroy { void operator()(mmd_unet_s* p) const { (void)mmd_unet_destroy(p); } };
  std::unique_ptr<mmd_unet_s, Destroy> u(new mmd_unet_s());
  u->T = n_diffusion_steps;
  u->precision = precision;
  if (options && options->two_per_workgroup_max != 0) u->ns2_max = options->two_per_workgroup_max < 0 ? 0 : options->two_per_workgroup_max;
  if (layered_path) {
    if (int rc = layered_create(&u->layered, s, n_diffusion_steps, tensors, options, st)) return rc;
  } else {
    std::vector<float> blob;
    pack_unet(s, tensors, n_diffusion_steps, blob, u->w);
    if (hipMalloc(&u->blob, blob.size() * sizeof(float)) != hipSuccess ||
        hipMalloc(&u->ttable, (size_t)u->T * u->w.tb_total * sizeof(float)) != hipSuccess) {
      set_error("mmd_unet_create: hipMalloc failed");
      return 1;
    }
    MMD_HIP_CHECK(hipMemcpyAsync(u->blob, blob.data(), blob.size() * sizeof(float), hipMemcpyHostToDevice, st));
    MMD_HIP_CHECK(hipStreamSynchronize(st));
    u->blob_bytes = blob.size() * sizeof(float);
    if (int rc = fill_time_table(u.get(), s, st)) return rc;
  }
  *out = u.release();
// ... 40 lines not shown
```

### mmd_amd/csrc/unet_kernel.h

```cpp
#pragma once
#include <hip/hip_runtime.h>

#include <cmath>
#include <cstdlib>
#include <cstring>
#include <type_traits>
#include <vector>

#include "../../include/mmd_amd.h"
#include "../../include/mmd_amd_debug.h"
#include "common.h"
#include "f16x2.h"
#include "gn_mish.h"
#include "guide_dev.h"
#include "unet_spec.h"

#ifdef MMD_UNET_F16
#define MMD_LO(...)
namespace mmd {
namespace f16 {
constexpr int N_PIECES = 1;
struct F16Pair { unsigned hi; };
__device__ __forceinline__ F16Pair f16_split2(float v0, float v1) {
  return F16Pair{__builtin_bit_cast(unsigned, __builtin_convertvector(f32x2{v0, v1}, f16x2))};
}
template <bool ZERO>
__device__ __forceinline__ void vb_three(f32x4& x, const u32x4 (&a)[2], const u32x4 (&b)[2]) {
  const f32x4 z = {0.f, 0.f, 0.f, 0.f};
  x = mfma_h(a[0], b[0], ZERO ? z : x);
  __builtin_amdgcn_sched_barrier(0);
}
#else
#define MMD_LO(...) __VA_ARGS__
namespace mmd {
constexpr int N_PIECES = 2;
#endif

struct FinalArgs {
  float* out;
  const uint4* w5;
  const float* isc;
  const float* bias;
  const float* gamma;
  const float* beta;
  float act;
  const uint4* w1_bf;
  const float* is1;
  const float* w1_bias;
};

template <int NT> struct Epi { float b[NT], g[NT], be[NT], is[NT], tb[NT]; };
template <int NT>
__device__ __forceinline__ Epi<NT> epi_load(const float* b, const float* g, const float* be, const float* tb, const float* isc, int c0) {
  Epi<NT> e;
#pragma unroll
  for (int t = 0; t < NT; ++t) {
    e.b[t] = b[c0 + t];
    e.g[t] = g[c0 + t];
    e.be[t] = be[c0 + t];
    e.is[t] = isc ? isc[c0 + t] : 1.f;
    e.tb[t] = tb ? tb[c0 + t] : 0.f;
  }
  return e;
}

struct RowPair { float a, b; };
__device__ __forceinline__ RowPair rows_xor16(float v) {
  const unsigned u = __builtin_bit_cast(unsigned, v);
  const auto r = __builtin_amdgcn_permlane16_swap(u, u, false, false);
  return RowPair{__builtin_bit_cast(float, (unsigned)r[0]), __builtin_bit_cast(float, (unsigned)r[1])};
}
__device__ __forceinline__ RowPair rows_xor32(float v) {
  const unsigned u = __builtin_bit_cast(unsigned, v);
  const auto r = __builtin_amdgcn_permlane32_swap(u, u, false, false);
  return RowPair{__builtin_bit_cast(float, (unsigned)r[0]), __builtin_bit_cast(float, (unsigned)r[1])};
}
__device__ __forceinline__ float add_xor16(float v) { const RowPair r = rows_xor16(v); return r.a + r.b; }
__device__ __forceinline__ float add_xor32(float v) { const RowPair r = rows_xor32(v); return r.a + r.b; }
__device__ __forceinline__ float max_nn(float a, float b) {
  const unsigned ua = __builtin_bit_cast(unsigned, a), ub = __builtin_bit_cast(unsigned, b);
  return __builtin_bit_cast(float, __builtin_elementwise_max(ua, ub));
}
__device__ __forceinline__ float max_xor16(float v) { const RowPair r = rows_xor16(v); return max_nn(r.a, r.b); }
__device__ __forceinline__ float max_xor32(float v) { const RowPair r = rows_xor32(v); return max_nn(r.a, r.b); }

template <int CTRL>
__device__ __forceinline__ float dpp_max(float v) {
  return max_nn(v, __builtin_bit_cast(float, __builtin_amdgcn_update_dpp(0, __builtin_bit_cast(int, v), CTRL, 0xF, 0xF, true)));
}
__device__ __forceinline__ float row_max16(float v) {
  v = dpp_max<0xB1>(v);
  v = dpp_max<0x4E>(v);
  v = dpp_max<0x141>(v);
  v = dpp_max<0x140>(v);
  return v;
}
__device__ __forceinline__ float wave_max(float v) {
// ... 1336 lines not shown
  for (int sm = 0; sm < NS; ++sm) s.sc[sm] = dyn_scale(mx_read(mx, sm)).s;
#pragma unroll
  for (int sl = 0; sl < NS / 2; ++sl) s.skip[sl] = dyn_scale(mx_read(mx, NS / 2 * (wave >> 1) + sl));
  return s;
}
template <int NS>
__device__ __forceinline__ void u1_store_chunk0(char* lb, int wave, int n, int g, const f32x4 (&xe)[NS][1], const f32x4 (&xo)[NS][1],
                                                const float (&sc)[NS]) {
  using GA = U1::GA;
  const bool odd = n & 1;
  char* const d0 = lb + wave * GA::G + (n >> 3) * GA::BX + ((n & 7) >> 1) * 4 + 2 * 16 + (8 * g + (odd ? 1 : 0)) * 16;
#pragma unroll
  for (int sm = 0; sm < NS; ++sm)
#pragma unroll
    for (int r = 0; r < 4; ++r) {
      const float own = (odd ? xo[sm][0][r] : xe[sm][0][r]) * sc[sm];
      const float recv = lane_swap1((odd ? xe[sm][0][r] : xo[sm][0][r]) * sc[sm]);
      const F16Pair p = f16_split2(odd ? recv : own, odd ? own : recv);
      char* d = d0 + sm * U1::W_BYTES + 2 * r * 16;
      *reinterpret_cast<unsigned*>(d) = p.hi;
      MMD_LO(*reinterpret_cast<unsigned*>(d + GA::PS) = p.lo;)
    }
}
template <int NS>
__device__ __forceinline__ void u1_store_chunk1(char* lb, int wave, int n, int g, const f32x4 (&skip)[NS][2], const DynScale (&sc)[NS / 2]) {
  using GA = U1::GA;
  const int np = wave & 1, s0 = NS / 2 * (wave >> 1);
  char* const sdst = lb + (2 * np + (n >> 3)) * GA::G + ((n >> 2) & 1) * GA::BX + (n & 3) * 4 + (2 + 4 * g) * 16;
#pragma unroll
  for (int m = 0; m < NS; ++m)
#pragma unroll
    for (int r = 0; r < 4; ++r) {
      const F16Pair p = f16_split2(skip[m][0][r] * sc[m >> 1].s, skip[m][1][r] * sc[m >> 1].s);
      char* d = sdst + (s0 + (m >> 1)) * U1::W_BYTES + (16 * (m & 1) + r) * 16;
      *reinterpret_cast<unsigned*>(d) = p.hi;
      MMD_LO(*reinterpret_cast<unsigned*>(d + GA::PS) = p.lo;)
    }
}
template <int MT>
__device__ __forceinline__ void u1_tail_store(char* vsF, int m0, int g, const f32x4 (&e)[MT][2], const f32x4 (&o)[MT][2], float s) {
  using GF [[maybe_unused]] = U1::GF;
#pragma unroll
  for (int mt = 0; mt < MT; ++mt)
#pragma unroll
    for (int r = 0; r < 4; ++r) {
      const F16Pair pe = f16_split2(e[mt][0][r] * s, e[mt][1][r] * s), po = f16_split2(o[mt][0][r] * s, o[mt][1][r] * s);
      char* d = vsF + (2 + 32 * (m0 + mt) + 8 * g + 2 * r) * 16;
      *reinterpret_cast<unsigned*>(d) = pe.hi;
      MMD_LO(*reinterpret_cast<unsigned*>(d + GF::PS) = pe.lo;)
      *reinterpret_cast<unsigned*>(d + 16) = po.hi;
      MMD_LO(*reinterpret_cast<unsigned*>(d + 16 + GF::PS) = po.lo;)
    }
}
template <int MT>
__device__ __forceinline__ void u1_eps_to_slab(float* et, int m0, int n, int g, const f32x4 (&out)[MT][1], float s1, float b1) {
  if (n < 4) {
#pragma unroll
    for (int mt = 0; mt < MT; ++mt)
#pragma unroll
      for (int r = 0; r < 4; ++r) et[(16 * (m0 + mt) + 4 * g + r) * 4 + n] = fmaf(out[mt][0][r], s1, b1);
  }
}
template <int MT>
__device__ __forceinline__ void u1_store_out(float* eps, size_t smp, int m0, int n, int g, const f32x4 (&out)[MT][1], float s1, float b1) {
  float* dst = eps + (smp * 64 + 16 * m0 + 4 * g) * 4 + n;
#pragma unroll
  for (int mt = 0; mt < MT; ++mt)
#pragma unroll
    for (int r = 0; r < 4; ++r) dst[(16 * mt + r) * 4] = fmaf(out[mt][0][r], s1, b1);
}
__device__ __forceinline__ void fused_ddpm_row(const FusedStep& fs, const float* et, int smp, int lane) {
  const float4 e = *reinterpret_cast<const float4*>(et + lane * 4);
  const int traj = fs.traj0 + smp, robot = traj / fs.spr;
  const size_t idx = (size_t)traj * H + lane;
  float4 v = ddpm_posterior_mean(fs.x[idx], e, fs.a_t, fs.b_t, fs.c1, fs.c2);
  if (fs.do_noise)
    v = add_step_noise(v, fs.noise ? fs.noise[idx] : traj_normal4(fs.seed, fs.robot_seeds, fs.draw, fs.traj_base, idx, robot, fs.spr), fs.sigma,
                       fs.noise_std_extra);
  float4 hv;
  if (hard_row(fs.hard_rows, fs.n_hard, fs.hard, robot, lane, hv)) v = hv;
  fs.x[idx] = v;
  if (fs.chain) fs.chain[idx] = v;
}

template <int NS>
__device__ __forceinline__ void chain_body_u1w(const ChainArgs& a, const FinalArgs& f, const FusedStep& fs, float* lds, int n0, int lane_in, int wave,
                                               const f32x4 (&xe)[NS][1], const f32x4 (&xo)[NS][1], const f32x4 (&skip)[NS][2],
                                               int trb, int tb_off = 0) {
  int lane = lane_in;
  asm volatile("" : "+v"(lane));
  using GA = U1::GA;
  using GB = U1::GB;
  using GF = U1::GF;
  constexpr int RDA = U1::RDA;
  char* const lb = reinterpret_cast<char*>(lds);
  char* const slab = lb + wave * U1::W_BYTES;
  float* const mx = lds + MX_OFF;
  const int n = lane & 15, g = lane >> 4, c0 = 2 * n;
  auto wt2 = [&](const uint4* w, int frags) { return w_tiles<2>(w, frags, 0, lane); };
  const WTiles<2> wp0 = wt2(a.r0.wa_bf, GA::FRAGS5), wp1 = wt2(a.wa0_c1_bf, GA::FRAGS5);
  const WTiles<2> wr0 = wt2(a.wres_bf, 2 * GA::KC), wr1 = wt2(a.wres_c1_bf, 2 * GA::KC);
  u32x4 ring[RDA][2][2];
  rd_ring_load<GA, 2, RDA>(ring, wp0);
  pair_maxima_out<2, 4>(skip, mx, wave, lane);
  __syncthreads();
  TR(trb + 0);
  const U1Scales<NS> sc = u1_input_scales<NS>(mx, wave);
  const float inv_in = dyn_scale(mx_read(mx, wave)).inv;
  rw_zero_halo<GA>(slab, 32, lane, true);
  u1_store_chunk0(lb, wave, n, g, xe, xo, sc.sc);
  TR(trb + 6);
  __syncthreads();
  TR(trb + 7);
  const char* const vaA = slab + g * GA::G + n * 16;
  f32x4 acc[2][2], res[2][2];
  rd_taps<GA, 2, 0, 5, true, true, 2, RDA>(acc, res, vaA, wp0, wr0, ring);
  rd_ring_load<GA, 2, RDA>(ring, wp1);
  TR(trb + 8);
  __syncthreads();
  u1_store_chunk1(lb, wave, n, g, skip, sc.skip);
  __syncthreads();
  TR(trb + 10);
  const Epi<2> e0a = epi_a<2>(a.r0, tb_off, c0);
  const float br[2] = {a.br[c0], a.br[c0 + 1]}, isr[2] = {a.isr[c0], a.isr[c0 + 1]};
  rd_taps<GA, 2, 0, 5, false, true, 2, RDA>(acc, res, vaA, wp1, wr1, ring);
  TR(trb + 11);
  const char* const vaB = slab + g * GB::G + n * 16;
  char* const vsB = slab + (n >> 2) * GB::G + (2 + 4 * g) * 16 + (n & 3) * 4;
  u32x4 ring5[5][2][2];
  auto preload = [&](const uint4* w) { rd_ring_load<GB, 2, 5>(ring5, wt2(w, GB::FRAGS5)); };
  preload(a.r0.wb_bf);
  auto conv = [&](const uint4* w) {
    const WTiles<2> wp = wt2(w, GB::FRAGS5);
    rw_store2<GB, 2>(vsB, acc);
    wave_lds_fence();
    rd_taps<GB, 2, 0, 5, true, false, 2, 5>(acc, res, vaB, wp, wp, ring5);
    wave_lds_fence();
  };
  tile_finish_res(res, isr, inv_in, br);
  rw_gn<2, 128>(acc, e0a, inv_in, a.r0.act_a);
  TR(trb + 1);
  wave_lds_fence();
  rw_zero_halo<GB>(slab, 32, lane, true);
  {
    const Epi<2> e = epi_b<2>(a.r0, c0);
    conv(a.r0.wb_bf);
    preload(a.ri[0].wa_bf);
    rw_gn<2, 128>(acc, e, 1.f, res);
  }
  TR(trb + 2);
  {
    const RtbPtrs& R = a.ri[0];
    tile_copy(res, acc);
    const DynScale ds = dyn_scale(rw_absmax(acc));
    tile_scale(acc, ds.s);
    const Epi<2> ea = epi_a<2>(R, tb_off, c0);
    conv(R.wa_bf);
    preload(R.wb_bf);
    rw_gn<2, 128>(acc, ea, ds.inv, R.act_a);
    TR(trb + 3);
    const Epi<2> eb = epi_b<2>(R, c0);
    conv(R.wb_bf);
    rw_gn<2, 128>(acc, eb, 1.f, res);
    TR(trb + 4);
  }
  const char* const vaF = slab + g * GF::G + n * 16;
  char* const vsF = slab + (n >> 2) * GF::G + (n & 3) * 4;
  f32x4 y[4][2];
  float inv_f;
  {
    const DynScale ds = dyn_scale(rw_absmax(acc));
    tile_scale(acc, ds.s);
    const WTiles<2> wt0 = wt2(a.wt_bf0, 2 * GB::KC * 2), wt1 = wt2(a.wt_bf1, 2 * GB::KC * 2);
    u32x4 ring2[2][2][2];
    const float bt[2] = {a.bt[c0], a.bt[c0 + 1]};
    const float is0[2] = {a.ist0[c0] * ds.inv, a.ist0[c0 + 1] * ds.inv}, is1[2] = {a.ist1[c0] * ds.inv, a.ist1[c0 + 1] * ds.inv};
    rd_ring_load<GB, 2, 2>(ring2, wt0);
    rw_store2<GB, 2>(vsB, acc);
    wave_lds_fence();
    f32x4 e[2][2], o[2][2];
    rd_taps<GB, 2, 1, 2, true, false, 2, 2>(e, res, vaB, wt0, wt0, ring2);
    rd_ring_load<GB, 2, 2>(ring2, wt1);
    rd_taps<GB, 2, 2, 2, true, false, 2, 2>(o, res, vaB, wt1, wt1, ring2);
    const DynScale df = dyn_scale(tail_up_epilogue(e, o, is0, is1, bt));
    inv_f = df.inv;
    wave_lds_fence();
    rw_zero_halo<GF>(slab, 64, lane, true);
    u1_tail_store<2>(vsF, 0, g, e, o, df.s);
  }
  TR(trb + 5);
  {
    const WTiles<2> wf = wt2(f.w5, GF::FRAGS5);
    rd_ring_load<GF, 2, 5>(ring5, wf);
    const WTiles<1> w1 = w_tiles<1>(f.w1_bf, 2 * GF::KC, 0, lane);
    u32x4 ring1[1][1][2];
    rd_ring_load<GF, 1, 1>(ring1, w1);
    const Epi<2> ef = epi_load<2>(f.bias, f.gamma, f.beta, nullptr, f.isc, c0);
    const float b1 = f.w1_bias[n & 3], s1 = f.is1[n & 3];
    wave_lds_fence();
    rd_taps<GF, 2, 0, 5, true, false, 4, 5>(y, y, vaF, wf, wf, ring5);
    rw_gn_mish_whole<4, 2, 2, 256, true>(y, ef.b, ef.g, ef.be, ef.is, inv_f, act_scale(f.act), [](int, int, int) { return 0.f; });
    wave_lds_fence();
    rw_store2<GF, 4>(vsF + (2 + 4 * g) * 16, y);
    wave_lds_fence();
    f32x4 out[4][1];
    rd_taps<GF, 1, 2, 1, true, false, 4, 1>(out, out, vaF, w1, w1, ring1);
    auto valid = [&] { return wave < NS && n0 + wave < a.n; };
    if (fs.enabled) {
      float* const et = reinterpret_cast<float*>(slab);
      wave_lds_fence();
      u1_eps_to_slab<4>(et, 0, n, g, out, s1, b1);
      wave_lds_fence();
      if (valid()) fused_ddpm_row(fs, et, n0 + wave, lane);
    } else if (n < 4 && valid()) {
      u1_store_out<4>(f.out, n0 + wave, 0, n, g, out, s1, b1);
    }
  }
}

template <int NV>
__device__ __forceinline__ void chain_body_u1s(const ChainArgs& a, const FinalArgs& f, const FusedStep& fs, float* lds, int n0, int lane_in, int wave,
                                               const f32x4 (&xe)[2][1], const f32x4 (&xo)[2][1], const f32x4 (&skip)[2][2], int trb, int tb_off = 0) {
  int lane = lane_in;
  asm volatile("" : "+v"(lane));
  using GA = U1::GA;
  using GB = U1::GB;
  using GF = U1::GF;
  constexpr int RDA = U1::RDA, TF = U1::TF;
  char* const lb = reinterpret_cast<char*>(lds);
  const int sp = wave >> 1, hf = wave & 1;
  char* const slab = lb + sp * U1::W_BYTES;
  float* const mx = lds + MX_OFF;
  const RwHalf half{reinterpret_cast<HalfStat*>(lds + PARK2_OFF) + sp * 128, hf, lane};
  const int n = lane & 15, g = lane >> 4, c0 = 2 * n;
  auto wt2 = [&](const uint4* w, int frags) { return w_tiles<2>(w, frags, 0, lane); };
  const WTiles<2> wp0 = wt2(a.r0.wa_bf, GA::FRAGS5), wp1 = wt2(a.wa0_c1_bf, GA::FRAGS5);
  const WTiles<2> wr0 = wt2(a.wres_bf, 2 * GA::KC), wr1 = wt2(a.wres_c1_bf, 2 * GA::KC);
  u32x4 ring[RDA][2][2];
  rd_ring_load<GA, 2, RDA>(ring, wp0);
  pair_maxima_out<2, 4>(skip, mx, wave, lane);
  __syncthreads();
  TR(trb + 0);
  char* const wb0 = lb + 2 * U1::W_BYTES;
  char* const wb1 = wb0 + WBUF_BYTES;
  stage_weights<2 * GB::FRAGS5>(a.r0.wb_bf, wb0, wave, lane);
  const U1Scales<2> sc = u1_input_scales<2>(mx, wave);
  const float inv_in = sc.skip[0].inv;
  rw_zero_halo<GA>(slab, 32, lane, hf == 0);
  u1_store_chunk0(lb, wave, n, g, xe, xo, sc.sc);
  TR(trb + 6);
  __syncthreads();
  TR(trb + 7);
  const char* const vaA = slab + g * GA::G + (n + 16 * hf) * 16;
  f32x4 acc[1][2], res[1][2];
  rd_taps<GA, 2, 0, 5, true, true, 1, RDA>(acc, res, vaA, wp0, wr0, ring);
  rd_ring_load<GA, 2, RDA>(ring, wp1);
  TR(trb + 8);
  __syncthreads();
  u1_store_chunk1(lb, wave, n, g, skip, sc.skip);
  __syncthreads();
  TR(trb + 10);
  const Epi<2> e0a = epi_a<2>(a.r0, tb_off, c0);
  const float br[2] = {a.br[c0], a.br[c0 + 1]}, isr[2] = {a.isr[c0], a.isr[c0 + 1]};
  rd_taps<GA, 2, 0, 5, false, true, 1, RDA>(acc, res, vaA, wp1, wr1, ring);
  TR(trb + 11);
  const char* const vaB = slab + g * GB::G + (n + 16 * hf) * 16;
  char* const vsB = slab + (n >> 2) * GB::G + (2 + 4 * g + 16 * hf) * 16 + (n & 3) * 4;
  u32x4 ring2[2][2][2];
  auto conv = [&](char* wb, auto stage_next) {
    const WStaged<2> wp = w_staged<2>(wb, GB::FRAGS5, lane);
    rw_store2<GB, 1>(vsB, acc);
    staged_weights_landed();
    __syncthreads();
    stage_next();
    rd_ring_load<GB, 2, 2>(ring2, wp);
    rd_taps<GB, 2, 0, 5, true, false, 1, 2>(acc, res, vaB, wp, wp, ring2);
  };
  tile_finish_res(res, isr, inv_in, br);
  rw_gn<2, 128>(acc, e0a, inv_in, a.r0.act_a, half);
  TR(trb + 1);
  rw_zero_halo<GB>(slab, 32, lane, hf == 0);
  {
    const Epi<2> e = epi_b<2>(a.r0, c0);
    conv(wb0, [&] { stage_weights<2 * GB::FRAGS5>(a.ri[0].wa_bf, wb1, wave, lane); });
    rw_gn<2, 128>(acc, e, 1.f, res, half);
  }
  TR(trb + 2);
  {
    const RtbPtrs& R = a.ri[0];
    tile_copy(res, acc);
    const DynScale ds = dyn_scale(half_sample_max(mx, sp, hf, lane, rw_absmax(acc)));
    tile_scale(acc, ds.s);
    const Epi<2> ea = epi_a<2>(R, tb_off, c0);
    conv(wb1, [&] { stage_weights<2 * GB::FRAGS5>(R.wb_bf, wb0, wave, lane); });
    rw_gn<2, 128>(acc, ea, ds.inv, R.act_a, half);
    TR(trb + 3);
    const Epi<2> eb = epi_b<2>(R, c0);
    conv(wb0, [&] {
      stage_weights<TF>(a.wt_bf0, wb1, wave, lane);
      stage_weights<TF>(a.wt_bf1, wb1 + TF * 1024, wave, lane);
    });
    rw_gn<2, 128>(acc, eb, 1.f, res, half);
    TR(trb + 4);
  }
  const char* const vaF = slab + g * GF::G + (n + 32 * hf) * 16;
  char* const vsF = slab + (n >> 2) * GF::G + (n & 3) * 4;
  f32x4 y[2][2];
  float inv_f;
  {
    const DynScale ds = dyn_scale(half_sample_max(mx, sp, hf, lane, rw_absmax(acc)));
    tile_scale(acc, ds.s);
    const WStaged<2> wt0 = w_staged<2>(wb1, TF / 2, lane), wt1 = w_staged<2>(wb1 + TF * 1024, TF / 2, lane);
    const float bt[2] = {a.bt[c0], a.bt[c0 + 1]};
    const float is0[2] = {a.ist0[c0] * ds.inv, a.ist0[c0 + 1] * ds.inv}, is1[2] = {a.ist1[c0] * ds.inv, a.ist1[c0 + 1] * ds.inv};
    rw_store2<GB, 1>(vsB, acc);
    staged_weights_landed();
    __syncthreads();
    stage_weights<2 * GF::FRAGS5>(f.w5, wb0, wave, lane);
    f32x4 e[1][2], o[1][2];
    rd_ring_load<GB, 2, 2>(ring2, wt0);
    rd_taps<GB, 2, 1, 2, true, false, 1, 2>(e, res, vaB, wt0, wt0, ring2);
    rd_ring_load<GB, 2, 2>(ring2, wt1);
    rd_taps<GB, 2, 2, 2, true, false, 1, 2>(o, res, vaB, wt1, wt1, ring2);
    const float m = tail_up_epilogue(e, o, is0, is1, bt);
    const DynScale df = dyn_scale(half_sample_max(mx, sp, hf, lane, m));
    inv_f = df.inv;
    rw_zero_halo<GF>(slab, 64, lane, hf == 0);
    u1_tail_store<1>(vsF, hf, g, e, o, df.s);
  }
  TR(trb + 5);
  {
    const WStaged<2> wf = w_staged<2>(wb0, GF::FRAGS5, lane);
    const WTiles<1> w1 = w_tiles<1>(f.w1_bf, 2 * GF::KC, 0, lane);
    u32x4 ring1[1][1][2];
    rd_ring_load<GF, 1, 1>(ring1, w1);
    const Epi<2> ef = epi_load<2>(f.bias, f.gamma, f.beta, nullptr, f.isc, c0);
    const float b1 = f.w1_bias[n & 3], s1 = f.is1[n & 3];
    staged_weights_landed();
    __syncthreads();
    rd_ring_load<GF, 2, 2>(ring2, wf);
    rd_taps<GF, 2, 0, 5, true, false, 2, 2>(y, y, vaF, wf, wf, ring2);
    rw_gn_mish_half<2, 2, 2, 256, true>(y, ef.b, ef.g, ef.be, ef.is, inv_f, act_scale(f.act), [](int, int, int) { return 0.f; }, half.xch, hf, lane);
    rw_store2<GF, 2>(vsF + (2 + 4 * g + 32 * hf) * 16, y);
    wave_lds_fence();
    f32x4 out[2][1];
    rd_taps<GF, 1, 2, 1, true, false, 2, 1>(out, out, vaF, w1, w1, ring1);
    auto valid = [&] { return sp < NV && n0 + sp < a.n; };
    if (fs.enabled) {
      float* const et = reinterpret_cast<float*>(slab);
      __syncthreads();
      u1_eps_to_slab<2>(et, 2 * hf, n, g, out, s1, b1);
      __syncthreads();
      if (hf == 0 && valid()) fused_ddpm_row(fs, et, n0 + sp, lane);
    } else if (n < 4 && valid()) {
      u1_store_out<2>(f.out, n0 + sp, 2 * hf, n, g, out, s1, b1);
    }
  }
}

struct UnetArgs {
  ChainArgs c[5];
  FinalArgs fin;
  int n;
  FusedStep fs;
};

template <int NS>
__device__ __forceinline__ void unet_forward_body(const UnetArgs& a, const FusedStep& fs, int tb_off, float* lds, int n0, int lane, int wave) {
  constexpr int NP = NS == 1 ? 2 : NS;
  f32x4 skip1[NP][2], skip2[NS][2], xe[NP][1], xo[NP][1];
  if constexpr (NS == 1) {
#pragma unroll
    for (int r = 0; r < 4; ++r) xe[1][0][r] = xo[1][0][r] = 0.f;
  }
  if constexpr (NS <= 2) chain_body_d0s<NS>(a.c[0], lds, n0, lane, wave, 0, tb_off);
  else chain_body_d0w<NS>(a.c[0], lds, n0, lane, wave, 0, tb_off);
  chain_body_d1d<NP>(a.c[1], lds, lane, wave, skip1, 40, tb_off);
  f32x4 mid_out[NS][2];
  chain_body_d2d<NS>(a.c[2], lds, lane, wave, mid_out, skip2, 80, tb_off);
  TR(130);
  {
    using G128 = RdGeo<128>;
    char* const slab128 = reinterpret_cast<char*>(lds) + D2::SLAB_OFF;
    char* const vs = slab128 + wave * G128::G + ((lane & 15) >> 2) * G128::BX + (2 + 4 * (lane >> 4)) * 16 + (lane & 3) * 4;
    chain_body_u0d<NS>(a.c[3], lds, lane, wave, mid_out, skip2, [&](const f32x4 (&t)[NS][2]) { rd_store2<G128>(vs, t); }, slab128,
                       sub_tile<NS>(xe, 0), sub_tile<NS>(xo, 0), 136, tb_off);
  }
  TR(131);
  if constexpr (NS <= 2) chain_body_u1s<NS>(a.c[4], a.fin, fs, lds, n0, lane, wave, xe, xo, skip1, 146, tb_off);
  else chain_body_u1w<NS>(a.c[4], a.fin, fs, lds, n0, lane, wave, xe, xo, skip1, 146, tb_off);
  TR(133);
}

template <int NS>
__global__ __launch_bounds__(256) __attribute__((amdgpu_waves_per_eu(2, 2))) void unet_kernel(UnetArgs a) {
  __shared__ __attribute__((aligned(16))) float lds[UNET_LDS_FLOATS];
  const int lane = threadIdx.x & 63;
  const int wave = __builtin_amdgcn_readfirstlane(threadIdx.x >> 6);
  unet_forward_body<NS>(a, a.fs, 0, lds, blockIdx.x * NS, lane, wave);
}

static_assert(sizeof(UnetArgs) <= PERSIST_TABLE_BYTES - PERSIST_ARGS_OFF, "the argument block fits its workspace region");
template <int NS>
__global__ __launch_bounds__(256) __attribute__((amdgpu_waves_per_eu(2, 2))) void unet_persist_kernel(const UnetArgs* ap, const FusedStep* steps,
                                                                                                     int n_steps, int tb_total) {
  __shared__ __attribute__((aligned(16))) float lds[UNET_LDS_FLOATS];
  const int lane = threadIdx.x & 63;
  const int wave = __builtin_amdgcn_readfirstlane(threadIdx.x >> 6);
  typedef const __attribute__((address_space(4))) UnetArgs* ConstArgs;
  typedef const __attribute__((address_space(4))) FusedStep* ConstStep;
  for (int s = 0; s < n_steps; ++s) {
    unsigned long long pa = reinterpret_cast<unsigned long long>(ap), ps = reinterpret_cast<unsigned long long>(steps + s);
    asm volatile("" : "+s"(pa), "+s"(ps));
    const UnetArgs& a = *(const UnetArgs*)(ConstArgs)pa;
    const FusedStep& fs = *(const FusedStep*)(ConstStep)ps;
    int lane_s = lane;
    asm volatile("" : "+v"(lane_s));
    unet_forward_body<NS>(a, fs, fs.t_row * tb_total, lds, blockIdx.x * NS, lane_s, wave);
    __threadfence_block();
    __syncthreads();
  }
}

#ifdef MMD_UNET_F16
}
#endif
}
```

Baseline: 96490.

## Fuse guide gradient iterations into the UNet kernel tail for guided steps

Adds an opt-in sampler flag (MMD_SAMPLER_FUSED_GUIDE) that runs the guided DDPM step inside the fp32, four-sample-per-block UNet kernel epilogue. The epilogue applies the model update, loads each robot's constraint slots into registers, then runs the guide iterations, noise and store. The guide device code moves into a shared header so both kernels can use it. This removes the separate guided-step kernel launch and the eps round trip through global memory on guided denoise steps. In exchange the UNet kernel gets a heavier tail that may raise register pressure, and the path only applies under its preconditions: no cons bins, samples_per_robot divisible by 4, slot count within capacity, f32 precision and a large enough chunk.

```diff
diff --git a/include/mmd_amd.h b/include/mmd_amd.h
--- a/include/mmd_amd.h
+++ b/include/mmd_amd.h
@@ -123,6 +123,7 @@
   const uint64_t* robot_seeds_dev;
 } mmd_sampler_desc;
 #define MMD_SAMPLER_NO_FUSED_STEP 1u
+#define MMD_SAMPLER_FUSED_GUIDE 4u
 #define MMD_SAMPLER_PERSIST 2u
 
 size_t mmd_sampler_workspace_bytes(mmd_unet_t unet, int n_traj);
diff --git a/mmd_amd/_lib.py b/mmd_amd/_lib.py
--- a/mmd_amd/_lib.py
+++ b/mmd_amd/_lib.py
@@ -56,7 +56,7 @@
     ]
 
 
-SAMPLER_NO_FUSED_STEP, SAMPLER_PERSIST = 1, 2
+SAMPLER_NO_FUSED_STEP, SAMPLER_PERSIST, SAMPLER_FUSED_GUIDE = 1, 2, 4
 UNET_LAYERED, UNET_LAYERED_VALU = 1, 2
 UNET_PRECISION_F32, UNET_PRECISION_F16 = 0, 1
 UNET_PRECISIONS = {"f32": UNET_PRECISION_F32, "f16": UNET_PRECISION_F16}
diff --git a/mmd_amd/csrc/api.hip b/mmd_amd/csrc/api.hip
--- a/mmd_amd/csrc/api.hip
+++ b/mmd_amd/csrc/api.hip
@@ -136,6 +136,26 @@
   fs.chain = reinterpret_cast<float4*>(chain); fs.hard = reinterpret_cast<const float4*>(hard);
   fs.t_row = t_row;
   return fs;
+}
+
+static FusedGuide fused_guide(const StepDev& sd, const GuideDev& g) {
+  FusedGuide fg{};
+  fg.enabled = 1;
+  fg.n_guide_steps = sd.n_guide_steps;
+  fg.grad_scale = sd.grad_scale;
+  fg.g = g;
+  return fg;
+}
+
+constexpr int kTailSlotsCompact = 64, kTailSlotsGeneral = 32;
+
+static bool guided_tail_allowed(mmd_unet_t unet, const mmd_sampler_desc* s, const mmd_guide_desc* guide, const GuideDev& g,
+                                const mmd_cons_bins* bins, int samples_per_robot) {
+  if (!guide || bins || !(s->flags & MMD_SAMPLER_FUSED_GUIDE) || (s->flags & MMD_SAMPLER_NO_FUSED_STEP) || !unet_fused_step_supported(unet)) return false;
+  if (samples_per_robot % 4 != 0) return false;
+  if (!g.robot_grp_off) return true;
+  const int cap = g.uniform_r2 > 0.f ? kTailSlotsCompact : kTailSlotsGeneral;
+  return guide->max_slots_per_robot > 0 && guide->max_slots_per_robot <= cap;
 }
 
 static int bins_of(const mmd_guide_desc* guide, const mmd_sampler_desc* s, const mmd_cons_bins** out) {
@@ -278,21 +298,27 @@
     MMD_HIP_CHECK(hipEventRecord(S->fork, st));
     for (int c = 0; c < nch; ++c) MMD_HIP_CHECK(hipStreamWaitEvent(cs[c], S->fork, 0));
   }
+  const bool guided_tail = guided_tail_allowed(unet, s, guide, g, bins, samples_per_robot);
   int rc = 0, k = k_start;
   for (int i = n_steps - 1 - k_start; i >= -n_steps_without_noise && rc == 0; --i, ++k) {
     StepDev sd{};
     if ((rc = make_step(s, i, guide != nullptr, sd))) break;
     sd.seed = seed; sd.draw = (unsigned int)k;
-    const bool fused = !sd.do_guide && !no_fused_step && unet_fused_step_supported(unet);
+    const bool plain_fused = !sd.do_guide && !no_fused_step && unet_fused_step_supported(unet);
     const float* noise_k = row_of(step_noise_dev, k, traj_floats);
     float* chain_k = row_of(chain_dev, k + 1, traj_floats);
+    bool fused[kMaxChunks];
     for (int c = 0; c < nch && rc == 0; ++c) {
       const int t0 = r0[c] * samples_per_robot, nc = (r0[c + 1] - r0[c]) * samples_per_robot;
+      const bool tail = sd.do_guide && guided_tail && unet_fused_guide_supported(unet, nc) && nc > guide_coop_limit(sd.coop_max);
+      fused[c] = plain_fused || tail;
+      const FusedGuide fg = tail ? fused_guide(sd, g) : FusedGuide{};
       rc = unet_forward_fused(unet, x_dev + (size_t)t0 * H * D, i < 0 ? 0 : i, eps + (size_t)t0 * H * D, nc, workspace_dev, uws, prof, cs[c],
-                              fused ? fused_step(sd, x_dev, hard_dev, noise_k, chain_k, t0, samples_per_robot) : FusedStep{});
-      if (fused) prof_skip(prof, 1);
-    }
-    for (int c = 0; c < nch && rc == 0 && !fused; ++c) {
+                              fused[c] ? fused_step(sd, x_dev, hard_dev, noise_k, chain_k, t0, samples_per_robot) : FusedStep{}, &fg);
+      if (fused[c]) prof_skip(prof, 1);
+    }
+    for (int c = 0; c < nch && rc == 0; ++c) {
+      if (fused[c]) continue;
       const int t0 = r0[c] * samples_per_robot, nc = (r0[c + 1] - r0[c]) * samples_per_robot;
       const bool br = prof_begin(prof, 1, sd.do_guide ? MMD_PROF_STEP_GUIDED : MMD_PROF_STEP_PLAIN, cs[c]);
       launch_step(g, sd, x_dev, eps, noise_k, chain_k, hard_dev, t0, nc, samples_per_robot, cs[c], bins);
diff --git a/mmd_amd/csrc/guide.hip b/mmd_amd/csrc/guide.hip
--- a/mmd_amd/csrc/guide.hip
+++ b/mmd_amd/csrc/guide.hip
@@ -12,254 +12,12 @@
 #include "bins_dev.h"
 #include "common.h"
 #include "guide_dev.h"
+#include "guide_step_dev.h"
 
 namespace mmd {
-
-__device__ __forceinline__ float clip_scale(float gx, float gy, float gz, float gw, float max_norm) {
-  const float ax = gx + 1e-6f, ay = gy + 1e-6f, az = gz + 1e-6f, aw = gw + 1e-6f;
-  const float n2 = ax * ax + ay * ay + az * az + aw * aw;
-  return fminf(max_norm * __builtin_amdgcn_rsqf(n2), 1.f);
-}
-
-__device__ __forceinline__ bool clip_grad(const GuideDev& g, float& gx, float& gy, float& gz, float& gw) {
-  if (g.clip_rule == 0) {
-    const float sc = clip_scale(gx, gy, gz, gw, g.max_norm);
-    gx = sc * gx; gy = sc * gy; gz = sc * gz; gw = sc * gw;
-    return sc < 1.f;
-  } else if (g.clip_rule == 1) {
-    const float m = g.max_value;
-    const bool on = fabsf(gx) > m || fabsf(gy) > m || fabsf(gz) > m || fabsf(gw) > m;
-    gx = fminf(fmaxf(gx, -m), m); gy = fminf(fmaxf(gy, -m), m); gz = fminf(fmaxf(gz, -m), m); gw = fminf(fmaxf(gw, -m), m);
-    return on;
-  }
-  return false;
-}
-__device__ __forceinline__ bool clip_grad(const GuideDev& g, float& gx, float& gy) {
-  float z = 0.f, w = 0.f;
-  return clip_grad(g, gx, gy, z, w);
-}
-
-__device__ __forceinline__ float lane_prev(float v) {
-  return __builtin_bit_cast(float, __builtin_amdgcn_update_dpp(0, __builtin_bit_cast(int, v), 0x138, 0xf, 0xf, true));
-}
-__device__ __forceinline__ float lane_next(float v) {
-  return __builtin_bit_cast(float, __builtin_amdgcn_update_dpp(0, __builtin_bit_cast(int, v), 0x130, 0xf, 0xf, true));
-}
 
 constexpr int LDS_SLOTS_SMALL = 40;
 constexpr int LDS_SLOTS_MAX = 144;
-
-__device__ __forceinline__ float rsq_pos(float d2) { return __builtin_amdgcn_rsqf(fmaxf(d2, 1e-30f)); }
-
-typedef float f32x2g __attribute__((ext_vector_type(2)));
-struct Acc4 { f32x2g a0, a1, a2, a3; };
-__device__ __forceinline__ Acc4 acc4_zero() {
-  const f32x2g z = {0.f, 0.f};
-  return Acc4{z, z, z, z};
-}
-__device__ __forceinline__ f32x2g acc4_total(const Acc4& r) {
-  return f32x2g{(r.a0.x + r.a1.x) + (r.a2.x + r.a3.x), (r.a0.y + r.a1.y) + (r.a2.y + r.a3.y)};
-}
-__device__ __forceinline__ f32x2g cons_term(f32x2g a, f32x2g p, f32x2g q, float r2) {
-  const float dx = p.x - q.x, dy = p.y - q.y;
-  const float d2 = __builtin_fmaf(dx, dx, dy * dy);
-  const float m = (d2 > r2) ? 0.f : rsq_pos(d2);
-  return f32x2g{__builtin_fmaf(-dx, m, a.x), __builtin_fmaf(-dy, m, a.y)};
-}
-template <bool COMPACT> struct ConsTab;
-template <> struct ConsTab<false> {
-  const float4* tab;
-  float r2;
-  __device__ __forceinline__ f32x2g add(f32x2g a, f32x2g p, int slot, int t) const {
-    const float4 c = tab[slot * H + t];
-    return cons_term(a, p, f32x2g{c.x, c.y}, c.w);
-  }
-};
-template <> struct ConsTab<true> {
-  const float2* tab;
-  float r2;
-  __device__ __forceinline__ f32x2g add(f32x2g a, f32x2g p, int slot, int t) const {
-    const float2 c = tab[slot * H + t];
-    return cons_term(a, p, f32x2g{c.x, c.y}, r2);
-  }
-};
-template <class TAB>
-__device__ __forceinline__ void cons_accumulate4(Acc4& acc, const TAB& tab, int first, int n, int rel, int t, f32x2g p) {
-  auto one = [&](int k, int slot) {
-    if (k == 0) acc.a0 = tab.add(acc.a0, p, slot, t);
-    else if (k == 1) acc.a1 = tab.add(acc.a1, p, slot, t);
-    else if (k == 2) acc.a2 = tab.add(acc.a2, p, slot, t);
-    else acc.a3 = tab.add(acc.a3, p, slot, t);
-  };
-  int i = 0;
-  for (; i < n && ((rel + i) & 3); ++i) one((rel + i) & 3, first + i);
-#pragma unroll 2
-  for (; i + 3 < n; i += 4) {
-    acc.a0 = tab.add(acc.a0, p, first + i, t);
-    acc.a1 = tab.add(acc.a1, p, first + i + 1, t);
-    acc.a2 = tab.add(acc.a2, p, first + i + 2, t);
-    acc.a3 = tab.add(acc.a3, p, first + i + 3, t);
-  }
-  for (int k = 0; i < n; ++i, ++k) one(k, first + i);
-}
-template <class TAB>
-__device__ __forceinline__ f32x2g cons_accumulate1(f32x2g a, const TAB& tab, int first, int n, int rel, int k, int t, f32x2g p) {
-#pragma unroll 4
-  for (int j = (k - rel) & 3; j < n; j += 4) a = tab.add(a, p, first + j, t);
-  return a;
-}
-
-struct GroupMeta {
-  static constexpr bool kOneGroup = false;
-  int s0[2], s1[2];
-  float w[2];
-  int grp0, n;
-  __device__ __forceinline__ void load(const GuideDev& g, int g0, int g1) {
-    grp0 = g0;
-    n = min(g1 - g0, 2);
-#pragma unroll
-    for (int k = 0; k < 2; ++k) {
-      s0[k] = s1[k] = 0;
-      w[k] = 0.f;
-      if (k < n) {
-        s0[k] = __builtin_amdgcn_readfirstlane(g.grp_slot_off[g0 + k]);
-        s1[k] = __builtin_amdgcn_readfirstlane(g.grp_slot_off[g0 + k + 1]);
-        w[k] = __builtin_bit_cast(float, __builtin_amdgcn_readfirstlane(__builtin_bit_cast(int, g.grp_weight[g0 + k])));
-      }
-    }
-  }
-  __device__ __forceinline__ void bounds(const GuideDev& g, int grp, int& a, int& b) const {
-    const int k = grp - grp0;
-    if (k == 0 && n > 0) { a = s0[0]; b = s1[0]; }
-    else if (k == 1 && n > 1) { a = s0[1]; b = s1[1]; }
-    else { a = __builtin_amdgcn_readfirstlane(g.grp_slot_off[grp]); b = __builtin_amdgcn_readfirstlane(g.grp_slot_off[grp + 1]); }
-  }
-  __device__ __forceinline__ float weight(const GuideDev& g, int grp) const {
-    const int k = grp - grp0;
-    return (k == 0 && n > 0) ? w[0] : (k == 1 && n > 1) ? w[1] : g.grp_weight[grp];
-  }
-};
-
-template <bool DUMP = false, class GROUPSUM, class GROUPW>
-__device__ __forceinline__ float4 guide_grad(const GuideDev& g, float4 xn, int t, const float4* __restrict__ grid,
-                                             int grp0, int grp1, GROUPSUM group_sum, GROUPW group_weight, unsigned int* tr = nullptr) {
-  unsigned int flags = 0;
-  float xu[4];
-  const float xv[4] = {xn.x, xn.y, xn.z, xn.w};
-#pragma unroll
-  for (int d = 0; d < 4; ++d) {
-    float v = fminf(fmaxf(xv[d], -1.f), 1.f);
-    if constexpr (DUMP) flags |= (fabsf(xv[d]) > 1.f ? 1u : 0u) << (16 + d);
-    v = (v + 1.f) / 2.f;
-    xu[d] = v * g.nscale[d] + g.nmin[d];
-  }
-  const float px = xu[0], py = xu[1], vx = xu[2], vy = xu[3];
-  const bool interior = t > 0 && t < H - 1;
-
-  int ix = (int)floorf((px - g.lo[0]) / g.dim[0] * (float)g.nx);
-  int iy = (int)floorf((py - g.lo[1]) / g.dim[1] * (float)g.ny);
-  ix = min(max(ix, 0), g.nx - 1);
-  iy = min(max(iy, 0), g.ny - 1);
-  const float4 cell0 = g.n_grids > 0 ? grid[(size_t)ix * g.ny + iy] : make_float4(1e30f, 0.f, 0.f, 0.f);
-
-  float wsx, wsy;
-  {
-    const float d0 = px - g.ws_min[0], d1 = py - g.ws_min[1], d2 = g.ws_max[0] - px, d3 = g.ws_max[1] - py;
-    float best = fmaxf(g.margin - d0, 0.f), gx = -1.f, gy = 0.f;
-    float v = fmaxf(g.margin - d1, 0.f);
-    if (v > best) { best = v; gx = 0.f; gy = -1.f; }
-    v = fmaxf(g.margin - d2, 0.f);
-    if (v > best) { best = v; gx = 1.f; gy = 0.f; }
-    v = fmaxf(g.margin - d3, 0.f);
-    if (v > best) { best = v; gx = 0.f; gy = 1.f; }
-    if (!(best > 0.f)) { gx = 0.f; gy = 0.f; }
-    if constexpr (DUMP) {
-      const unsigned arg = gx < 0.f ? 0u : gy < 0.f ? 1u : gx > 0.f ? 2u : 3u;
-      if (best > 0.f) flags |= 1u << 4 | arg << 5;
-    }
-    const bool clipped = clip_grad(g, gx, gy);
-    if constexpr (DUMP) flags |= (clipped ? 1u : 0u) << 9;
-    wsx = g.w_coll * gx; wsy = g.w_coll * gy;
-  }
-  float gpx, gpy, gpz, gpw;
-  {
-    const float npx = lane_next(px), npy = lane_next(py), nvx = lane_next(vx), nvy = lane_next(vy);
-    float wpx = 0.f, wpy = 0.f, wvx = 0.f, wvy = 0.f;
-    if (t < H - 1) {
-      const float epx = npx - (px + g.dt * vx), epy = npy - (py + g.dt * vy);
-      const float evx = nvx - vx, evy = nvy - vy;
-      wpx = 2.f * (g.m1 * epx + g.m2 * evx);
-      wpy = 2.f * (g.m1 * epy + g.m2 * evy);
-      wvx = 2.f * (g.m2 * epx + g.m3 * evx);
-      wvy = 2.f * (g.m2 * epy + g.m3 * evy);
-    }
-    const float lpx = lane_prev(wpx), lpy = lane_prev(wpy), lvx = lane_prev(wvx), lvy = lane_prev(wvy);
-    float gx = lpx - wpx, gy = lpy - wpy;
-    float gz = lvx - (g.dt * wpx + wvx), gw = lvy - (g.dt * wpy + wvy);
-    const bool clipped = clip_grad(g, gx, gy, gz, gw);
-    if constexpr (DUMP) flags |= (clipped ? 1u : 0u) << 10;
-    gpx = g.w_smooth * gx; gpy = g.w_smooth * gy;
-    gpz = g.w_smooth * gz; gpw = g.w_smooth * gw;
-  }
-  float cx = 0.f, cy = 0.f;
-  for (int grp = grp0; grp < grp1; ++grp) {
-    const f32x2g gs = group_sum(grp, f32x2g{px, py});
-    float gx = gs.x, gy = gs.y;
-    const bool clipped = clip_grad(g, gx, gy);
-    if constexpr (DUMP) {
-      const int k = grp - grp0, s0 = g.grp_slot_off[grp], s1 = g.grp_slot_off[grp + 1];
-      unsigned long long mask = 0;
-      unsigned int n_act = 0;
-      for (int sl = s0; sl < s1; ++sl) {
-        const float4 c = g.cons[(size_t)sl * H + t];
-        const float dx = px - c.x, dy = py - c.y;
-        const float d2 = __builtin_fmaf(dx, dx, dy * dy);
-        if (!(d2 > c.w)) {
-          ++n_act;
-          if (sl - s0 < 64) mask |= 1ull << (sl - s0);
-        }
-      }
-      if (k < 4) {
-        tr[2 + 2 * k] = (unsigned int)mask;
-        tr[3 + 2 * k] = (unsigned int)(mask >> 32);
-        flags |= (clipped ? 1u : 0u) << (11 + k);
-      }
-      tr[10] += n_act;
-    }
-    const float w = group_weight(grp);
-    cx += w * gx; cy += w * gy;
-  }
-  float ox, oy;
-  {
-    float best = fmaxf(g.margin - cell0.x, 0.f), gx = 0.f, gy = 0.f;
-    unsigned win = 0;
-    if (best > 0.f) { gx = -cell0.y; gy = -cell0.z; }
-    for (int k = 1; k < g.n_grids; ++k) {
-      const float4 c = grid[((size_t)k * g.nx + ix) * g.ny + iy];
-      const float v = fmaxf(g.margin - c.x, 0.f);
-      if (v > best) { best = v; gx = -c.y; gy = -c.z; win = (unsigned)k; }
-    }
-    if (g.n_xs + g.n_xb > 0) {
-      float ex, ey;
-      const float v = fmaxf(g.margin - extra_sdf(g.xs, g.n_xs, g.xb, g.n_xb, px, py, ex, ey), 0.f);
-      if (v > best) { best = v; gx = -ex; gy = -ey; win = 7u; }
-    }
-    const bool clipped = clip_grad(g, gx, gy);
-    if constexpr (DUMP) {
-      if (best > 0.f) flags |= 1u | (win & 7u) << 1;
-      flags |= (clipped ? 1u : 0u) << 8;
-    }
-    ox = g.w_coll * gx; oy = g.w_coll * gy;
-  }
-  if constexpr (DUMP) {
-    tr[0] = (unsigned int)(ix * g.ny + iy);
-    tr[1] = flags | (unsigned int)min(grp1 - grp0, 15) << 20;
-  }
-  float tx = ((ox + wsx) + gpx) + cx, ty = ((oy + wsy) + gpy) + cy;
-  float tz = gpz, tw = gpw;
-  if (!interior) { tx = ty = tz = tw = 0.f; }
-  return make_float4(-tx, -ty, -tz, -tw);
-}
 
 
 template <bool COMPACT, int NT>
@@ -290,51 +48,6 @@
   }
   const int g0 = lds_n > 0 ? max(s0, lds_slot0 + lds_n) : s0;
   if (s1 > g0) acc(ConsTab<false>{g.cons, 0.f}, g0, s1 - g0, g0 - s0);
-}
-
-__device__ __forceinline__ float4 model_update(StepDev s, float4 v, const float4* eps, size_t idx) {
-  if (s.do_model)
-    v = s.ddim == 2 ? ddim_update_x0(v, eps[idx], s.a_t, s.b_t, s.c1, s.c2)
-        : s.ddim ? ddim_update(v, eps[idx], s.a_t, s.b_t, s.c1, s.c2) : ddpm_posterior_mean(v, eps[idx], s.a_t, s.b_t, s.c1, s.c2);
-  return v;
-}
-
-template <bool DUMP, class META = GroupMeta, class GROUPSUM>
-__device__ __forceinline__ void guide_iterations(const GuideDev& g, const StepDev& s, int robot, int t, size_t idx, float4& v, bool is_hard,
-                                                 float4 hv, bool store, GROUPSUM group_sum) {
-  const int map = g.robot_map ? g.robot_map[robot] : 0;
-  const float4* grid = g.grids + (size_t)map * g.n_grids * g.nx * g.ny;
-  int grp0 = 0, grp1 = 0;
-  if constexpr (META::kOneGroup) {
-    grp1 = 1;
-  } else if (g.robot_grp_off) {
-    grp0 = __builtin_amdgcn_readfirstlane(g.robot_grp_off[robot]);
-    grp1 = __builtin_amdgcn_readfirstlane(g.robot_grp_off[robot + 1]);
-  }
-  META gm;
-  if constexpr (META::kOneGroup) gm.w = group_sum.weight;
-  gm.load(g, grp0, grp1);
-  for (int it = 0; it < s.n_guide_steps; ++it) {
-    unsigned int* tr = nullptr;
-    if constexpr (DUMP) {
-      tr = s.trace + ((size_t)it * s.guide_chain_stride + idx) * MMD_TRACE_WORDS;
-      for (int w = 0; w < MMD_TRACE_WORDS; ++w) tr[w] = 0u;
-    }
-    const float4 gr = guide_grad<DUMP>(g, v, t, grid, grp0, grp1, [&](int grp, f32x2g p) { return group_sum(gm, grp, p); },
-                                       [&](int grp) { return gm.weight(g, grp); }, tr);
-    v.x = __builtin_fmaf(s.grad_scale, gr.x, v.x); v.y = __builtin_fmaf(s.grad_scale, gr.y, v.y);
-    v.z = __builtin_fmaf(s.grad_scale, gr.z, v.z); v.w = __builtin_fmaf(s.grad_scale, gr.w, v.w);
-    if (is_hard) v = hv;
-    if (s.guide_chain && store) s.guide_chain[(size_t)it * s.guide_chain_stride + idx] = v;
-  }
-}
-
-__device__ __forceinline__ void step_finish(const StepDev& s, float4* x, const float4* noise, float4* chain, size_t idx, int robot,
-                                            int samples_per_robot, float4& v, bool is_hard, const float4& hv) {
-  if (s.do_noise) v = add_step_noise(v, noise ? noise[idx] : traj_normal4(s.seed, s.robot_seeds, s.draw, s.traj_base, idx, robot, samples_per_robot), s.sigma, s.noise_std_extra);
-  if (is_hard) v = hv;
-  x[idx] = v;
-  if (chain) chain[idx] = v;
 }
 
 template <int WPB, bool COMPACT, bool DUMP = false>
@@ -637,6 +350,7 @@
 }
 
 constexpr int kCoopMaxTrajDefault = 512;
+int guide_coop_limit(int coop_max) { return coop_max > 0 ? coop_max : coop_max < 0 ? 0 : kCoopMaxTrajDefault; }
 
 int launch_step(const GuideDev& g, StepDev s, float* x, const float* eps, const float* noise, float* chain,
                 const float* hard, int traj0, int n_traj, int spr, hipStream_t st, const mmd_cons_bins* bins) {
@@ -657,7 +371,7 @@
   };
   if (s.trace) {
     launch(ddpm_guide_kernel<4, false, true>, (n_traj + 3) / 4, 256, 0, 0);
-  } else if (guided && n_traj <= (s.coop_max > 0 ? s.coop_max : s.coop_max < 0 ? 0 : kCoopMaxTrajDefault)) {
+  } else if (guided && n_traj <= guide_coop_limit(s.coop_max)) {
     const int fit = 60 * 1024 / bytes_per_slot;
     const int slots = g.max_slots < fit ? g.max_slots : fit;
     launch(compact ? ddpm_guide_coop_kernel<true> : ddpm_guide_coop_kernel<false>, n_traj, 256,
diff --git a/mmd_amd/csrc/guide_dev.h b/mmd_amd/csrc/guide_dev.h
--- a/mmd_amd/csrc/guide_dev.h
+++ b/mmd_amd/csrc/guide_dev.h
@@ -36,7 +36,7 @@
   for (int i = 0; i < n_xs; ++i) {
     const float4 s = xs[i];
     const float dx = px - s.x, dy = py - s.y;
-    const float n = kTorchNorm ? sqrtf(__builtin_fmaf(dy, dy, dx * dx)) : sqrtf(dx * dx + dy * dy), d = n - s.z;
+    const float n = kTorchNorm ? sqrtf(__builtin_fmaf(dy, dy, dx * dx)) : sqrtf(__builtin_fmaf(dx, dx, dy * dy)), d = n - s.z;
     if (d < best) { best = d; gx = n > 0.f ? dx / n : 0.f; gy = n > 0.f ? dy / n : 0.f; }
   }
   for (int i = 0; i < n_xb; ++i) {
@@ -44,7 +44,7 @@
     const float rad = 0.3f * fminf(b.z, b.w);
     const float dx = px - b.x, dy = py - b.y, qx = fabsf(dx) - b.z + rad, qy = fabsf(dy) - b.w + rad;
     const float mq = fmaxf(qx, qy), rx = fmaxf(qx, 0.f), ry = fmaxf(qy, 0.f);
-    const float n = kTorchNorm ? sqrtf(__builtin_fmaf(ry, ry, rx * rx)) : sqrtf(rx * rx + ry * ry);
+    const float n = kTorchNorm ? sqrtf(__builtin_fmaf(ry, ry, rx * rx)) : sqrtf(__builtin_fmaf(rx, rx, ry * ry));
     const float d = fminf(mq, 0.f) + n - rad;
     if (d < best) {
       best = d;
@@ -132,6 +132,13 @@
   int t_row;
 };
 
+struct FusedGuide {
+  int enabled;
+  int n_guide_steps;
+  float grad_scale;
+  GuideDev g;
+};
+
 constexpr int PERSIST_MAX_STEPS = 64;
 constexpr int PERSIST_ARGS_OFF = 8192;
 constexpr int PERSIST_TABLE_BYTES = 12288;
@@ -167,14 +174,16 @@
 
 int fill_guide(const mmd_guide_desc* d, GuideDev& g);
 bool unet_fused_step_supported(mmd_unet_t u);
+bool unet_fused_guide_supported(mmd_unet_t u, int n);
 int unet_forward_fused(mmd_unet_t u, const float* x, int t, float* eps, int n, void* ws, size_t ws_bytes, Profiler* prof,
-                       hipStream_t st, const FusedStep& fs);
+                       hipStream_t st, const FusedStep& fs, const FusedGuide* fg = nullptr);
 int unet_persist_steps(mmd_unet_t u, int n, void* ws, size_t ws_bytes, hipStream_t st, const FusedStep* steps, int n_steps);
 int launch_unet_f16(int ns, int blocks, hipStream_t st, const void* args, size_t args_bytes);
 int launch_unet_persist_f16(int ns, int blocks, hipStream_t st, const void* args_dev, size_t args_bytes, const FusedStep* steps_dev,
                             int n_steps, int tb_total);
 int launch_step(const GuideDev& g, StepDev s, float* x, const float* eps, const float* noise, float* chain,
                 const float* hard, int traj0, int n_traj, int spr, hipStream_t st, const mmd_cons_bins* bins);
+int guide_coop_limit(int coop_max);
 int launch_init(float* x, float* chain, const float* hard, unsigned long long hard_rows, int draw, unsigned long long seed,
                 const unsigned long long* robot_seeds, long long traj_base, int n_traj, int spr, hipStream_t st);
 
diff --git a/mmd_amd/csrc/guide_step_dev.h b/mmd_amd/csrc/guide_step_dev.h
--- /dev/null
+++ b/mmd_amd/csrc/guide_step_dev.h
@@ -0,0 +1,357 @@
+#pragma once
+#include <hip/hip_runtime.h>
+
+#include "../../include/mmd_amd.h"
+#include "../../include/mmd_amd_debug.h"
+#include "common.h"
+#include "guide_dev.h"
+
+namespace mmd {
+
+__device__ __forceinline__ float clip_scale(float gx, float gy, float gz, float gw, float max_norm) {
+  const float ax = gx + 1e-6f, ay = gy + 1e-6f, az = gz + 1e-6f, aw = gw + 1e-6f;
+  const float n2 = __builtin_fmaf(ax, ax, ay * ay) + az * az + aw * aw;
+  return fminf(max_norm * __builtin_amdgcn_rsqf(n2), 1.f);
+}
+
+__device__ __forceinline__ bool clip_grad(const GuideDev& g, float& gx, float& gy, float& gz, float& gw) {
+  if (g.clip_rule == 0) {
+    const float sc = clip_scale(gx, gy, gz, gw, g.max_norm);
+    gx = sc * gx; gy = sc * gy; gz = sc * gz; gw = sc * gw;
+    return sc < 1.f;
+  } else if (g.clip_rule == 1) {
+    const float m = g.max_value;
+    const bool on = fabsf(gx) > m || fabsf(gy) > m || fabsf(gz) > m || fabsf(gw) > m;
+    gx = fminf(fmaxf(gx, -m), m); gy = fminf(fmaxf(gy, -m), m); gz = fminf(fmaxf(gz, -m), m); gw = fminf(fmaxf(gw, -m), m);
+    return on;
+  }
+  return false;
+}
+__device__ __forceinline__ bool clip_grad(const GuideDev& g, float& gx, float& gy) {
+  float z = 0.f, w = 0.f;
+  return clip_grad(g, gx, gy, z, w);
+}
+
+__device__ __forceinline__ float lane_prev(float v) {
+  return __builtin_bit_cast(float, __builtin_amdgcn_update_dpp(0, __builtin_bit_cast(int, v), 0x138, 0xf, 0xf, true));
+}
+__device__ __forceinline__ float lane_next(float v) {
+  return __builtin_bit_cast(float, __builtin_amdgcn_update_dpp(0, __builtin_bit_cast(int, v), 0x130, 0xf, 0xf, true));
+}
+
+__device__ __forceinline__ float rsq_pos(float d2) { return __builtin_amdgcn_rsqf(fmaxf(d2, 1e-30f)); }
+
+typedef float f32x2g __attribute__((ext_vector_type(2)));
+struct Acc4 { f32x2g a0, a1, a2, a3; };
+__device__ __forceinline__ Acc4 acc4_zero() {
+  const f32x2g z = {0.f, 0.f};
+  return Acc4{z, z, z, z};
+}
+__device__ __forceinline__ f32x2g acc4_total(const Acc4& r) {
+  return f32x2g{(r.a0.x + r.a1.x) + (r.a2.x + r.a3.x), (r.a0.y + r.a1.y) + (r.a2.y + r.a3.y)};
+}
+__device__ __forceinline__ f32x2g cons_term(f32x2g a, f32x2g p, f32x2g q, float r2) {
+  const float dx = p.x - q.x, dy = p.y - q.y;
+  const float d2 = __builtin_fmaf(dx, dx, dy * dy);
+  const float m = (d2 > r2) ? 0.f : rsq_pos(d2);
+  return f32x2g{__builtin_fmaf(-dx, m, a.x), __builtin_fmaf(-dy, m, a.y)};
+}
+template <bool COMPACT> struct ConsTab;
+template <> struct ConsTab<false> {
+  const float4* tab;
+  float r2;
+  __device__ __forceinline__ f32x2g add(f32x2g a, f32x2g p, int slot, int t) const {
+    const float4 c = tab[slot * H + t];
+    return cons_term(a, p, f32x2g{c.x, c.y}, c.w);
+  }
+};
+template <> struct ConsTab<true> {
+  const float2* tab;
+  float r2;
+  __device__ __forceinline__ f32x2g add(f32x2g a, f32x2g p, int slot, int t) const {
+    const float2 c = tab[slot * H + t];
+    return cons_term(a, p, f32x2g{c.x, c.y}, r2);
+  }
+};
+template <class TAB>
+__device__ __forceinline__ void cons_accumulate4(Acc4& acc, const TAB& tab, int first, int n, int rel, int t, f32x2g p) {
+  auto one = [&](int k, int slot) {
+    if (k == 0) acc.a0 = tab.add(acc.a0, p, slot, t);
+    else if (k == 1) acc.a1 = tab.add(acc.a1, p, slot, t);
+    else if (k == 2) acc.a2 = tab.add(acc.a2, p, slot, t);
+    else acc.a3 = tab.add(acc.a3, p, slot, t);
+  };
+  int i = 0;
+  for (; i < n && ((rel + i) & 3); ++i) one((rel + i) & 3, first + i);
+#pragma unroll 2
+  for (; i + 3 < n; i += 4) {
+    acc.a0 = tab.add(acc.a0, p, first + i, t);
+    acc.a1 = tab.add(acc.a1, p, first + i + 1, t);
+    acc.a2 = tab.add(acc.a2, p, first + i + 2, t);
+    acc.a3 = tab.add(acc.a3, p, first + i + 3, t);
+  }
+  for (int k = 0; i < n; ++i, ++k) one(k, first + i);
+}
+template <class TAB>
+__device__ __forceinline__ f32x2g cons_accumulate1(f32x2g a, const TAB& tab, int first, int n, int rel, int k, int t, f32x2g p) {
+#pragma unroll 4
+  for (int j = (k - rel) & 3; j < n; j += 4) a = tab.add(a, p, first + j, t);
+  return a;
+}
+
+template <bool COMPACT, int NSLOT>
+struct RegCons {
+  static_assert(NSLOT % 16 == 0, "loaded sixteen slots a batch");
+  float qx[NSLOT], qy[NSLOT], r2[COMPACT ? 1 : NSLOT];
+  int base, n;
+  __device__ __forceinline__ void load(const GuideDev& g, int slot0, int slots, int t) {
+    base = slot0;
+    n = min(slots, NSLOT);
+    if constexpr (COMPACT) r2[0] = g.uniform_r2;
+    const float4* const src = g.cons + (size_t)slot0 * H + t;
+#pragma unroll
+    for (int b = 0; b < NSLOT; b += 16) {
+      if (b < n) {
+        float4 c[16];
+#pragma unroll
+        for (int j = 0; j < 16; ++j) c[j] = src[(size_t)min(b + j, n - 1) * H];
+#pragma unroll
+        for (int j = 0; j < 16; ++j) {
+          if constexpr (COMPACT) {
+            qx[b + j] = c[j].z < 0.f ? 1e30f : c[j].x;
+            qy[b + j] = c[j].z < 0.f ? 1e30f : c[j].y;
+          } else {
+            qx[b + j] = c[j].x; qy[b + j] = c[j].y; r2[b + j] = c[j].w;
+          }
+        }
+      }
+    }
+  }
+  __device__ __forceinline__ f32x2g sum(const GuideDev& g, int s0, int s1, int t, f32x2g p) const {
+    const int a = min(s0 - base, n), b = min(s1 - base, n);
+    const f32x2g z = {0.f, 0.f};
+    f32x2g b0 = z, b1 = z, b2 = z, b3 = z;
+    float px = p.x, py = p.y;
+    auto term = [&](f32x2g acc, int j) { return cons_term(acc, f32x2g{px, py}, f32x2g{qx[j], qy[j]}, r2[COMPACT ? 0 : j]); };
+#pragma unroll
+    for (int j = 0; j < NSLOT; j += 4) {
+      if (j + 4 > a && j < b) {
+        if (j >= a && j + 4 <= b) {
+          b0 = term(b0, j); b1 = term(b1, j + 1); b2 = term(b2, j + 2); b3 = term(b3, j + 3);
+        } else {
+          if (j >= a) b0 = term(b0, j);
+          if (j + 1 >= a && j + 1 < b) b1 = term(b1, j + 1);
+          if (j + 2 >= a && j + 2 < b) b2 = term(b2, j + 2);
+          if (j + 3 < b) b3 = term(b3, j + 3);
+        }
+        float a0x = b0.x, a0y = b0.y, a1x = b1.x, a1y = b1.y, a2x = b2.x, a2y = b2.y, a3x = b3.x, a3y = b3.y;
+        asm volatile("" : "+v"(a0x), "+v"(a0y), "+v"(a1x), "+v"(a1y), "+v"(a2x), "+v"(a2y), "+v"(a3x), "+v"(a3y), "+v"(px), "+v"(py));
+        b0 = f32x2g{a0x, a0y}; b1 = f32x2g{a1x, a1y}; b2 = f32x2g{a2x, a2y}; b3 = f32x2g{a3x, a3y};
+      }
+    }
+    const int rot = a & 3;
+    Acc4 acc = rot == 0 ? Acc4{b0, b1, b2, b3} : rot == 1 ? Acc4{b1, b2, b3, b0} : rot == 2 ? Acc4{b2, b3, b0, b1} : Acc4{b3, b0, b1, b2};
+    const int o0 = max(s0, base + NSLOT);
+    if (s1 > o0) cons_accumulate4(acc, ConsTab<false>{g.cons, 0.f}, o0, s1 - o0, o0 - s0, t, p);
+    return acc4_total(acc);
+  }
+};
+
+struct GroupMeta {
+  static constexpr bool kOneGroup = false;
+  int s0[2], s1[2];
+  float w[2];
+  int grp0, n;
+  __device__ __forceinline__ void load(const GuideDev& g, int g0, int g1) {
+    grp0 = g0;
+    n = min(g1 - g0, 2);
+#pragma unroll
+    for (int k = 0; k < 2; ++k) {
+      s0[k] = s1[k] = 0;
+      w[k] = 0.f;
+      if (k < n) {
+        s0[k] = __builtin_amdgcn_readfirstlane(g.grp_slot_off[g0 + k]);
+        s1[k] = __builtin_amdgcn_readfirstlane(g.grp_slot_off[g0 + k + 1]);
+        w[k] = __builtin_bit_cast(float, __builtin_amdgcn_readfirstlane(__builtin_bit_cast(int, g.grp_weight[g0 + k])));
+      }
+    }
+  }
+  __device__ __forceinline__ void bounds(const GuideDev& g, int grp, int& a, int& b) const {
+    const int k = grp - grp0;
+    if (k == 0 && n > 0) { a = s0[0]; b = s1[0]; }
+    else if (k == 1 && n > 1) { a = s0[1]; b = s1[1]; }
+    else { a = __builtin_amdgcn_readfirstlane(g.grp_slot_off[grp]); b = __builtin_amdgcn_readfirstlane(g.grp_slot_off[grp + 1]); }
+  }
+  __device__ __forceinline__ float weight(const GuideDev& g, int grp) const {
+    const int k = grp - grp0;
+    return (k == 0 && n > 0) ? w[0] : (k == 1 && n > 1) ? w[1] : g.grp_weight[grp];
+  }
+};
+
+template <bool DUMP = false, class GROUPSUM, class GROUPW>
+__device__ __forceinline__ float4 guide_grad(const GuideDev& g, float4 xn, int t, const float4* __restrict__ grid,
+                                             int grp0, int grp1, GROUPSUM group_sum, GROUPW group_weight, unsigned int* tr = nullptr) {
+  unsigned int flags = 0;
+  float xu[4];
+  const float xv[4] = {xn.x, xn.y, xn.z, xn.w};
+#pragma unroll
+  for (int d = 0; d < 4; ++d) {
+    float v = fminf(fmaxf(xv[d], -1.f), 1.f);
+    if constexpr (DUMP) flags |= (fabsf(xv[d]) > 1.f ? 1u : 0u) << (16 + d);
+    v = (v + 1.f) / 2.f;
+    xu[d] = v * g.nscale[d] + g.nmin[d];
+  }
+  const float px = xu[0], py = xu[1], vx = xu[2], vy = xu[3];
+  const bool interior = t > 0 && t < H - 1;
+
+  int ix = (int)floorf((px - g.lo[0]) / g.dim[0] * (float)g.nx);
+  int iy = (int)floorf((py - g.lo[1]) / g.dim[1] * (float)g.ny);
+  ix = min(max(ix, 0), g.nx - 1);
+  iy = min(max(iy, 0), g.ny - 1);
+  const float4 cell0 = g.n_grids > 0 ? grid[(size_t)ix * g.ny + iy] : make_float4(1e30f, 0.f, 0.f, 0.f);
+
+  float wsx, wsy;
+  {
+    const float d0 = px - g.ws_min[0], d1 = py - g.ws_min[1], d2 = g.ws_max[0] - px, d3 = g.ws_max[1] - py;
+    float best = fmaxf(g.margin - d0, 0.f), gx = -1.f, gy = 0.f;
+    float v = fmaxf(g.margin - d1, 0.f);
+    if (v > best) { best = v; gx = 0.f; gy = -1.f; }
+    v = fmaxf(g.margin - d2, 0.f);
+    if (v > best) { best = v; gx = 1.f; gy = 0.f; }
+    v = fmaxf(g.margin - d3, 0.f);
+    if (v > best) { best = v; gx = 0.f; gy = 1.f; }
+    if (!(best > 0.f)) { gx = 0.f; gy = 0.f; }
+    if constexpr (DUMP) {
+      const unsigned arg = gx < 0.f ? 0u : gy < 0.f ? 1u : gx > 0.f ? 2u : 3u;
+      if (best > 0.f) flags |= 1u << 4 | arg << 5;
+    }
+    const bool clipped = clip_grad(g, gx, gy);
+    if constexpr (DUMP) flags |= (clipped ? 1u : 0u) << 9;
+    wsx = g.w_coll * gx; wsy = g.w_coll * gy;
+  }
+  float gpx, gpy, gpz, gpw;
+  {
+    const float npx = lane_next(px), npy = lane_next(py), nvx = lane_next(vx), nvy = lane_next(vy);
+    float wpx = 0.f, wpy = 0.f, wvx = 0.f, wvy = 0.f;
+    if (t < H - 1) {
+      const float epx = npx - (px + g.dt * vx), epy = npy - (py + g.dt * vy);
+      const float evx = nvx - vx, evy = nvy - vy;
+      wpx = 2.f * __builtin_fmaf(g.m1, epx, g.m2 * evx);
+      wpy = 2.f * __builtin_fmaf(g.m1, epy, g.m2 * evy);
+      wvx = 2.f * __builtin_fmaf(g.m2, epx, g.m3 * evx);
+      wvy = 2.f * __builtin_fmaf(g.m2, epy, g.m3 * evy);
+    }
+    const float lpx = lane_prev(wpx), lpy = lane_prev(wpy), lvx = lane_prev(wvx), lvy = lane_prev(wvy);
+    float gx = lpx - wpx, gy = lpy - wpy;
+    float gz = lvx - (g.dt * wpx + wvx), gw = lvy - (g.dt * wpy + wvy);
+    const bool clipped = clip_grad(g, gx, gy, gz, gw);
+    if constexpr (DUMP) flags |= (clipped ? 1u : 0u) << 10;
+    gpx = g.w_smooth * gx; gpy = g.w_smooth * gy;
+    gpz = g.w_smooth * gz; gpw = g.w_smooth * gw;
+  }
+  float cx = 0.f, cy = 0.f;
+  for (int grp = grp0; grp < grp1; ++grp) {
+    const f32x2g gs = group_sum(grp, f32x2g{px, py});
+    float gx = gs.x, gy = gs.y;
+    const bool clipped = clip_grad(g, gx, gy);
+    if constexpr (DUMP) {
+      const int k = grp - grp0, s0 = g.grp_slot_off[grp], s1 = g.grp_slot_off[grp + 1];
+      unsigned long long mask = 0;
+      unsigned int n_act = 0;
+      for (int sl = s0; sl < s1; ++sl) {
+        const float4 c = g.cons[(size_t)sl * H + t];
+        const float dx = px - c.x, dy = py - c.y;
+        const float d2 = __builtin_fmaf(dx, dx, dy * dy);
+        if (!(d2 > c.w)) {
+          ++n_act;
+          if (sl - s0 < 64) mask |= 1ull << (sl - s0);
+        }
+      }
+      if (k < 4) {
+        tr[2 + 2 * k] = (unsigned int)mask;
+        tr[3 + 2 * k] = (unsigned int)(mask >> 32);
+        flags |= (clipped ? 1u : 0u) << (11 + k);
+      }
+      tr[10] += n_act;
+    }
+    const float w = group_weight(grp);
+    cx += w * gx; cy += w * gy;
+  }
+  float ox, oy;
+  {
+    float best = fmaxf(g.margin - cell0.x, 0.f), gx = 0.f, gy = 0.f;
+    unsigned win = 0;
+    if (best > 0.f) { gx = -cell0.y; gy = -cell0.z; }
+    for (int k = 1; k < g.n_grids; ++k) {
+      const float4 c = grid[((size_t)k * g.nx + ix) * g.ny + iy];
+      const float v = fmaxf(g.margin - c.x, 0.f);
+      if (v > best) { best = v; gx = -c.y; gy = -c.z; win = (unsigned)k; }
+    }
+    if (g.n_xs + g.n_xb > 0) {
+      float ex, ey;
+      const float v = fmaxf(g.margin - extra_sdf(g.xs, g.n_xs, g.xb, g.n_xb, px, py, ex, ey), 0.f);
+      if (v > best) { best = v; gx = -ex; gy = -ey; win = 7u; }
+    }
+    const bool clipped = clip_grad(g, gx, gy);
+    if constexpr (DUMP) {
+      if (best > 0.f) flags |= 1u | (win & 7u) << 1;
+      flags |= (clipped ? 1u : 0u) << 8;
+    }
+    ox = g.w_coll * gx; oy = g.w_coll * gy;
+  }
+  if constexpr (DUMP) {
+    tr[0] = (unsigned int)(ix * g.ny + iy);
+    tr[1] = flags | (unsigned int)min(grp1 - grp0, 15) << 20;
+  }
+  float tx = ((ox + wsx) + gpx) + cx, ty = ((oy + wsy) + gpy) + cy;
+  float tz = gpz, tw = gpw;
+  if (!interior) { tx = ty = tz = tw = 0.f; }
+  return make_float4(-tx, -ty, -tz, -tw);
+}
+
+__device__ __forceinline__ float4 model_update(StepDev s, float4 v, const float4* eps, size_t idx) {
+  if (s.do_model)
+    v = s.ddim == 2 ? ddim_update_x0(v, eps[idx], s.a_t, s.b_t, s.c1, s.c2)
+        : s.ddim ? ddim_update(v, eps[idx], s.a_t, s.b_t, s.c1, s.c2) : ddpm_posterior_mean(v, eps[idx], s.a_t, s.b_t, s.c1, s.c2);
+  return v;
+}
+
+template <bool DUMP, class META = GroupMeta, class GROUPSUM>
+__device__ __forceinline__ void guide_iterations(const GuideDev& g, const StepDev& s, int robot, int t, size_t idx, float4& v, bool is_hard,
+                                                 float4 hv, bool store, GROUPSUM group_sum) {
+  const int map = g.robot_map ? g.robot_map[robot] : 0;
+  const float4* grid = g.grids + (size_t)map * g.n_grids * g.nx * g.ny;
+  int grp0 = 0, grp1 = 0;
+  if constexpr (META::kOneGroup) {
+    grp1 = 1;
+  } else if (g.robot_grp_off) {
+    grp0 = __builtin_amdgcn_readfirstlane(g.robot_grp_off[robot]);
+    grp1 = __builtin_amdgcn_readfirstlane(g.robot_grp_off[robot + 1]);
+  }
+  META gm;
+  if constexpr (META::kOneGroup) gm.w = group_sum.weight;
+  gm.load(g, grp0, grp1);
+  for (int it = 0; it < s.n_guide_steps; ++it) {
+    unsigned int* tr = nullptr;
+    if constexpr (DUMP) {
+      tr = s.trace + ((size_t)it * s.guide_chain_stride + idx) * MMD_TRACE_WORDS;
+      for (int w = 0; w < MMD_TRACE_WORDS; ++w) tr[w] = 0u;
+    }
+    const float4 gr = guide_grad<DUMP>(g, v, t, grid, grp0, grp1, [&](int grp, f32x2g p) { return group_sum(gm, grp, p); },
+                                       [&](int grp) { return gm.weight(g, grp); }, tr);
+    v.x = __builtin_fmaf(s.grad_scale, gr.x, v.x); v.y = __builtin_fmaf(s.grad_scale, gr.y, v.y);
+    v.z = __builtin_fmaf(s.grad_scale, gr.z, v.z); v.w = __builtin_fmaf(s.grad_scale, gr.w, v.w);
+    if (is_hard) v = hv;
+    if (s.guide_chain && store) s.guide_chain[(size_t)it * s.guide_chain_stride + idx] = v;
+  }
+}
+
+__device__ __forceinline__ void step_finish(const StepDev& s, float4* x, const float4* noise, float4* chain, size_t idx, int robot,
+                                            int samples_per_robot, float4& v, bool is_hard, const float4& hv) {
+  if (s.do_noise) v = add_step_noise(v, noise ? noise[idx] : traj_normal4(s.seed, s.robot_seeds, s.draw, s.traj_base, idx, robot, samples_per_robot), s.sigma, s.noise_std_extra);
+  if (is_hard) v = hv;
+  x[idx] = v;
+  if (chain) chain[idx] = v;
+}
+
+}
diff --git a/mmd_amd/csrc/unet.hip b/mmd_amd/csrc/unet.hip
--- a/mmd_amd/csrc/unet.hip
+++ b/mmd_amd/csrc/unet.hip
@@ -328,7 +328,7 @@
 }
 
 int unet_forward_fused(mmd_unet_t u, const float* x, int t, float* eps, int n, void* ws, size_t ws_bytes, Profiler* prof,
-                       hipStream_t st, const FusedStep& fs) {
+                       hipStream_t st, const FusedStep& fs, const FusedGuide* fg) {
   MMD_REQUIRE(u && x && eps && ws, "mmd_unet_forward: NULL argument");
   MMD_REQUIRE(n >= 1, "mmd_unet_forward: n_traj must be >= 1");
   MMD_REQUIRE(t >= 0 && t < u->T, "mmd_unet_forward: t=%d outside [0,%d)", t, u->T);
@@ -342,6 +342,10 @@
   }
   UnetArgs a = unet_args(u, x, t, n, eps);
   a.fs = fs;
+  if (fg && fg->enabled) {
+    MMD_REQUIRE(fs.enabled && unet_fused_guide_supported(u, n), "mmd_unet_forward: no guided tail in the kernel of this launch (%d trajectories)", n);
+    a.fg = *fg;
+  }
   const bool bracket = prof_begin(prof, 0, fs.enabled ? MMD_PROF_UNET_FUSED : MMD_PROF_UNET, st);
   int rc = 0;
   if (u->precision == MMD_UNET_PRECISION_F16) {
@@ -375,6 +379,9 @@
   return 0;
 }
 bool unet_fused_step_supported(mmd_unet_t u) { return u && !u->layered; }
+bool unet_fused_guide_supported(mmd_unet_t u, int n) {
+  return unet_fused_step_supported(u) && u->precision != MMD_UNET_PRECISION_F16 && n > u->ns2_max;
+}
 
 static constexpr double rtb_flops(double cin, double cout, double L) {
   return 2.0 * cout * 5 * cin * L + 2.0 * cout * 5 * cout * L + (cin != cout ? 2.0 * cout * cin * L : 0.0);
diff --git a/mmd_amd/csrc/unet_kernel.h b/mmd_amd/csrc/unet_kernel.h
--- a/mmd_amd/csrc/unet_kernel.h
+++ b/mmd_amd/csrc/unet_kernel.h
@@ -13,6 +13,7 @@
 #include "f16x2.h"
 #include "gn_mish.h"
 #include "guide_dev.h"
+#include "guide_step_dev.h"
 #include "unet_spec.h"
 
 #ifdef MMD_UNET_F16
@@ -1515,9 +1516,43 @@
   fs.x[idx] = v;
   if (fs.chain) fs.chain[idx] = v;
 }
-
-template <int NS>
-__device__ __forceinline__ void chain_body_u1w(const ChainArgs& a, const FinalArgs& f, const FusedStep& fs, float* lds, int n0, int lane_in, int wave,
+template <bool COMPACT, int NSLOT>
+__device__ __forceinline__ void fused_guide_iterations(const GuideDev& g, const StepDev& s, int robot, int lane, size_t idx, float4& v, bool is_hard,
+                                                       const float4& hv, int slot0, int slots) {
+  RegCons<COMPACT, NSLOT> rc;
+  rc.load(g, slot0, slots, lane);
+  guide_iterations<false>(g, s, robot, lane, idx, v, is_hard, hv, true, [&](const GroupMeta& gm, int grp, f32x2g p) {
+    int s0, s1;
+    gm.bounds(g, grp, s0, s1);
+    return rc.sum(g, s0, s1, lane, p);
+  });
+}
+__device__ __forceinline__ void fused_guided_row(const FusedStep& fs, const FusedGuide& fg, const float* et, int smp, int lane) {
+  const GuideDev& g = fg.g;
+  const int traj = fs.traj0 + smp, robot = traj / fs.spr;
+  const size_t idx = (size_t)traj * H + lane;
+  StepDev s{};
+  s.a_t = fs.a_t; s.b_t = fs.b_t; s.c1 = fs.c1; s.c2 = fs.c2; s.sigma = fs.sigma; s.noise_std_extra = fs.noise_std_extra;
+  s.grad_scale = fg.grad_scale;
+  s.do_model = 1; s.do_guide = 1; s.do_noise = fs.do_noise;
+  s.n_guide_steps = fg.n_guide_steps;
+  s.n_hard = fs.n_hard; s.hard_rows = fs.hard_rows;
+  s.seed = fs.seed; s.robot_seeds = fs.robot_seeds; s.draw = fs.draw; s.traj_base = fs.traj_base;
+  float4 v = model_update(s, fs.x[idx], reinterpret_cast<const float4*>(et), (size_t)lane);
+  float4 hv = v;
+  const bool is_hard = hard_row(s.hard_rows, s.n_hard, fs.hard, robot, lane, hv);
+  int slot0 = 0, slots = 0;
+  if (g.robot_grp_off) {
+    slot0 = __builtin_amdgcn_readfirstlane(g.grp_slot_off[g.robot_grp_off[robot]]);
+    slots = __builtin_amdgcn_readfirstlane(g.grp_slot_off[g.robot_grp_off[robot + 1]]) - slot0;
+  }
+  if (g.uniform_r2 > 0.f) fused_guide_iterations<true, 64>(g, s, robot, lane, idx, v, is_hard, hv, slot0, slots);
+  else fused_guide_iterations<false, 32>(g, s, robot, lane, idx, v, is_hard, hv, slot0, slots);
+  step_finish(s, fs.x, fs.noise, fs.chain, idx, robot, fs.spr, v, is_hard, hv);
+}
+
+template <int NS, bool GUIDED>
+__device__ __forceinline__ void chain_body_u1w(const ChainArgs& a, const FinalArgs& f, const FusedStep& fs, const FusedGuide& fg, float* lds, int n0, int lane_in, int wave,
                                                const f32x4 (&xe)[NS][1], const f32x4 (&xo)[NS][1], const f32x4 (&skip)[NS][2],
                                                int trb, int tb_off = 0) {
   int lane = lane_in;
@@ -1644,7 +1679,14 @@
       wave_lds_fence();
       u1_eps_to_slab<4>(et, 0, n, g, out, s1, b1);
       wave_lds_fence();
-      if (valid()) fused_ddpm_row(fs, et, n0 + wave, lane);
+      if (valid()) {
+        if constexpr (GUIDED) {
+          if (fg.enabled) fused_guided_row(fs, fg, et, n0 + wave, lane);
+          else fused_ddpm_row(fs, et, n0 + wave, lane);
+        } else {
+          fused_ddpm_row(fs, et, n0 + wave, lane);
+        }
+      }
     } else if (n < 4 && valid()) {
       u1_store_out<4>(f.out, n0 + wave, 0, n, g, out, s1, b1);
     }
@@ -1796,9 +1838,10 @@
   FinalArgs fin;
   int n;
   FusedStep fs;
+  FusedGuide fg;
 };
 
-template <int NS>
+template <int NS, bool GUIDED = false>
 __device__ __forceinline__ void unet_forward_body(const UnetArgs& a, const FusedStep& fs, int tb_off, float* lds, int n0, int lane, int wave) {
   constexpr int NP = NS == 1 ? 2 : NS;
   f32x4 skip1[NP][2], skip2[NS][2], xe[NP][1], xo[NP][1];
@@ -1821,7 +1864,7 @@
   }
   TR(131);
   if constexpr (NS <= 2) chain_body_u1s<NS>(a.c[4], a.fin, fs, lds, n0, lane, wave, xe, xo, skip1, 146, tb_off);
-  else chain_body_u1w<NS>(a.c[4], a.fin, fs, lds, n0, lane, wave, xe, xo, skip1, 146, tb_off);
+  else chain_body_u1w<NS, GUIDED>(a.c[4], a.fin, fs, a.fg, lds, n0, lane, wave, xe, xo, skip1, 146, tb_off);
   TR(133);
 }
 
@@ -1830,7 +1873,12 @@
   __shared__ __attribute__((aligned(16))) float lds[UNET_LDS_FLOATS];
   const int lane = threadIdx.x & 63;
   const int wave = __builtin_amdgcn_readfirstlane(threadIdx.x >> 6);
-  unet_forward_body<NS>(a, a.fs, 0, lds, blockIdx.x * NS, lane, wave);
+#ifdef MMD_UNET_F16
+  constexpr bool kGuidedTail = false;
+#else
+  constexpr bool kGuidedTail = NS == 4;
+#endif
+  unet_forward_body<NS, kGuidedTail>(a, a.fs, 0, lds, blockIdx.x * NS, lane, wave);
 }
 
 static_assert(sizeof(UnetArgs) <= PERSIST_TABLE_BYTES - PERSIST_ARGS_OFF, "the argument block fits its workspace region");
```

Result: slower. 95310 (-1.2%).
